# jlk9/MPAS-Ocean.jl

Measured on AMD Instinct MI355X. Metric: cell-updates/sec per RK4 step, higher is better.
Workload: dtype f64

## Files before the change

include/moka_hip.h:

```cpp
#ifndef MOKA_HIP_H
#define MOKA_HIP_H
#include <stdint.h>

#ifdef __cplusplus
extern "C" {
#endif

typedef struct moka_ctx   moka_ctx;
typedef struct moka_plan  moka_plan;
typedef struct moka_mesh  moka_mesh;
typedef struct moka_state moka_state;

typedef enum {
    MOKA_OK = 0,
    MOKA_ERR_ARG = -1,
    MOKA_ERR_HIP = -2,
    MOKA_ERR_NO_DEVICE = -3,
    MOKA_ERR_ALLOC = -4,
    MOKA_ERR_UNSUPPORTED = -5,
    MOKA_ERR_COMM = -6
} moka_status;

typedef enum {
    MOKA_ORDER_DEFAULT = 0,
// ... 112 lines not shown
int  moka_state_upload(moka_state *st, int field, int time_level, const double *host);
int  moka_state_download(moka_state *st, int field, int time_level, double *host);

int  moka_state_download_rows(moka_state *st, int field, int time_level, int64_t nRows, const int32_t *rows, double *host);

int  moka_state_array_address(moka_state *st, int field, int time_level, uint64_t *address);

int  moka_state_optimize_placement(moka_state *st, int max_tries, double *ms_before, double *ms_after);
typedef struct { int32_t field; double ms_old, ms_new; int32_t kept; } moka_placement_trial;
int  moka_state_placement_log(const moka_state *st, int32_t capacity, moka_placement_trial *out, int32_t *n);
int64_t moka_state_placement_launches(const moka_state *st);

int moka_advance_time_levels(moka_state *st, int flags);
int moka_diagnostic_compute(moka_state *st, int flags);
int moka_compute_normal_velocity_tendency(moka_state *st, int flags);
int moka_compute_layer_thickness_tendency(moka_state *st, int flags);
int moka_tendencies(moka_state *st);
int moka_step_fe(moka_state *st, double dt, int flags);
int moka_step_rk4(moka_state *st, double dt);
int moka_run(moka_state *st, int integrator, double dt, int64_t nsteps, int flags);
int moka_sum_sq(moka_state *st, int field, int time_level, double *out);

typedef struct moka_halo moka_halo;
int  moka_ctx_streams(moka_ctx *ctx, void **compute_stream, void **comm_stream);
int  moka_mesh_permutation(const moka_mesh *mesh, int kind, int32_t *new_to_old);
int  moka_mesh_class_ranges(const moka_mesh *mesh, int32_t capacity, int32_t *nClasses, int32_t *patchStart,
                            int32_t *cellStart, int32_t *edgeStart);
int  moka_halo_create(moka_state *st, int32_t nNeighbors, const int32_t *sendCells, const int64_t *sendCellOff,
                      const int32_t *sendEdges, const int64_t *sendEdgeOff, const int32_t *recvCells,
                      const int64_t *recvCellOff, const int32_t *recvEdges, const int64_t *recvEdgeOff,
                      int32_t nPatchesBoundary, int32_t nPatchesOwned, moka_halo **out);
void moka_halo_destroy(moka_halo *h);
int  moka_halo_buffer_elems(const moka_halo *h, int64_t *sendElems, int64_t *recvElems);
int  moka_halo_pack(moka_halo *h, int what, void *sendbuf_device);
int  moka_halo_unpack(moka_halo *h, int what, const void *recvbuf_device);

typedef struct {
    unsigned char ipc[15][64];
    uint64_t ptr[15];
    uint64_t flagPtr;
    char     shmName[64];
    int32_t  dstCell, dstEdge;
    int32_t  nCells, nEdges;
    int32_t  slot;
    int32_t  nNeighbors, pid, device, stateBytes, nVertLevels;
} moka_halo_peer_info;
int  moka_halo_set_overlap(moka_halo *h, int mode);
int  moka_halo_set_acquire(moka_halo *h, int on);
int  moka_halo_pack_fields(moka_halo *h, const void *uField, const void *hField, const void *sField, void *sendbuf);
int  moka_halo_unpack_fields(moka_halo *h, void *uField, void *hField, void *sField, const void *recvbuf);
int  moka_halo_direct_available(const moka_halo *h);
int  moka_halo_export(moka_halo *h, int32_t nbr, int32_t shared, moka_halo_peer_info *out);
int  moka_halo_connect(moka_halo *h, int32_t nbr, const moka_halo_peer_info *peer, int32_t shared);
int  moka_halo_push_begin(moka_halo *h, int what);
int  moka_halo_push_signal(moka_halo *h);
int  moka_halo_push_wait(moka_halo *h, double timeout_s);

int  moka_halo_set_stream_flags(moka_halo *h, int on);

typedef struct {
    int64_t steps, exchanges, boundary_launches, interior_launches;
    double host_step_ms, host_signal_wait_ms, host_flag_store_ms, host_wait_ms, boundary_launch_ms, interior_launch_ms;
} moka_halo_stats;
int  moka_halo_stats_enable(moka_halo *h, int on);
int  moka_halo_stats_read(moka_halo *h, moka_halo_stats *out);

int  moka_rk4_dist_begin(moka_halo *h, double dt);
int  moka_rk4_dist_stage(moka_halo *h, int stage, int part);
int  moka_rk4_dist_parts_available(const moka_halo *h);
int  moka_rk4_dist_stage_launch(moka_halo *h, int stage);
int  moka_rk4_dist_end(moka_halo *h);
typedef int (*moka_transport_fn)(void *user, int what, void *sendbuf_device, void *recvbuf_device);
int  moka_rk4_dist_step(moka_halo *h, double dt, moka_transport_fn transport, void *user, void *sendbuf_device,
                        void *recvbuf_device, double timeout_s);
int  moka_fe_dist_launch(moka_halo *h, double dt, int flags, int part);
int  moka_fe_dist_end(moka_halo *h);
int  moka_fe_dist_step(moka_halo *h, double dt, int flags, moka_transport_fn transport, void *user, void *sendbuf_device,
                       void *recvbuf_device, double timeout_s);

int moka_kernel_variant_available(int variant);
int moka_set_kernel_variant(moka_ctx *ctx, int variant);
int moka_set_tuning(int key, int value);
int moka_get_tuning(int key, int *value);
int moka_state_rk4_streams(const moka_state *st);
int moka_stage_timing(moka_ctx *ctx, int enable);
int moka_stage_timing_read(moka_ctx *ctx, double ms[4], int64_t *steps);
int moka_ctx_pci_bus_id(moka_ctx *ctx, char *buf, int32_t len);
int moka_mark(moka_ctx *ctx);
int moka_marks_reset(moka_ctx *ctx);
int moka_marks_read(moka_ctx *ctx, int64_t capacity, double *ms, int64_t *n);
int moka_bw_probe(moka_ctx *ctx, int64_t bytes, int iters, double gbs[4]);
int moka_bw_probe_streams(moka_ctx *ctx, int iters, double *gbs);
int moka_bw_probe_reread(moka_ctx *ctx, int64_t region, int reps, int iters, double *gbs);
int moka_bw_probe_gather_big(moka_ctx *ctx, int64_t bytes, int iters, double *gbs);
int moka_last_fe_path(const moka_state *st);
int moka_fe_lazy_pending(const moka_state *st);

int  moka_set_nonlinear(moka_state *st, int on);
int  moka_set_viscosity_del2(moka_state *st, double viscDel2);
int  moka_set_viscosity_del4(moka_state *st, double viscDel4, const double *meshScalingDel4);
int  moka_state_del4_path(const moka_state *st);

int  moka_set_tracers(moka_state *st, int32_t nTracers);
int  moka_tracer_upload(moka_state *st, int32_t j, int time_level, const double *host);
int  moka_tracer_download(moka_state *st, int32_t j, int time_level, double *host);
int  moka_state_tracer_path(const moka_state *st);
int  moka_set_tracer_diffusion(moka_state *st, const double *kappa);
int  moka_tracer_diffusion(const moka_state *st, int32_t j, double *out);
int  moka_set_tracer_biharmonic(moka_state *st, const double *kappa4);
int  moka_tracer_biharmonic(const moka_state *st, int32_t j, double *out);
int  moka_tracer_source_upload(moka_state *st, int32_t j, const double *host);
int  moka_tracer_source_download(moka_state *st, int32_t j, double *host);
int  moka_tracer_has_source(const moka_state *st, int32_t j, int *out);
int  moka_set_tracer_vertical_diffusion(moka_state *st, const double *kappaV);
int  moka_tracer_vertical_diffusion(const moka_state *st, int32_t j, double *out);
int  moka_state_tracer_vmix_path(const moka_state *st);
int  moka_tracer_vertical_field_upload(moka_state *st, int32_t j, const double *host);
int  moka_tracer_vertical_field_download(moka_state *st, int32_t j, double *host);
int  moka_tracer_has_vertical_field(const moka_state *st, int32_t j, int *out);

int  moka_set_vertical_viscosity(moka_state *st, double nuV, double bottomDrag);
int  moka_vertical_viscosity(const moka_state *st, double *nuV, double *bottomDrag);
int  moka_surface_stress_upload(moka_state *st, const double *host);
int  moka_surface_stress_download(moka_state *st, double *host);
int  moka_has_surface_stress(const moka_state *st, int *out);
int  moka_state_momentum_vmix_path(const moka_state *st);
int  moka_vertical_viscosity_field_upload(moka_state *st, const double *host);
int  moka_vertical_viscosity_field_download(moka_state *st, double *host);
int  moka_has_vertical_viscosity_field(const moka_state *st, int *out);

typedef struct moka_tracer_tape moka_tracer_tape;
int  moka_tracer_tape_create(moka_state *st, int64_t capacity_steps, moka_tracer_tape **out);
void moka_tracer_tape_destroy(moka_tracer_tape *t);
int  moka_step_rk4_tracer_taped(moka_tracer_tape *t, double dt);
int  moka_tracer_tape_steps(const moka_tracer_tape *t, int64_t *n);
int  moka_tracer_adjoint_seed(moka_tracer_tape *t, int32_t j, const double *host);
int  moka_tracer_adjoint_sweep(moka_tracer_tape *t);
int  moka_tracer_adjoint_download(moka_tracer_tape *t, int32_t j, double *host);
int  moka_tracer_adjoint_path(const moka_tracer_tape *t);
int  moka_tracer_adjoint_vmix_path(const moka_tracer_tape *t);
int  moka_tracer_adjoint_want_source_gradient(moka_tracer_tape *t, int32_t j, int on);
int  moka_tracer_adjoint_source_download(moka_tracer_tape *t, int32_t j, double *host);
enum { MOKA_TRACER_GRAD_KAPPA = 1, MOKA_TRACER_GRAD_KAPPA4 = 2 };
int  moka_tracer_adjoint_want_diffusivity_gradient(moka_tracer_tape *t, int32_t j, int what, int on);
int  moka_tracer_adjoint_diffusivity_gradient(moka_tracer_tape *t, int32_t j, int what, double *out);
int  moka_tracer_adjoint_diffusivity_density_download(moka_tracer_tape *t, int32_t j, int what, double *host);
int  moka_tracer_adjoint_want_vertical_gradient(moka_tracer_tape *t, int32_t j, int on);
int  moka_tracer_adjoint_vertical_gradient(moka_tracer_tape *t, int32_t j, double *out);
enum { MOKA_VGRAD_INTERFACE = 0, MOKA_VGRAD_CELL = 1, MOKA_VGRAD_PROFILE = 2 };
int  moka_tracer_adjoint_vertical_density_download(moka_tracer_tape *t, int32_t j, int view, double *host);

typedef struct moka_tape moka_tape;
int  moka_tape_create(moka_state *st, int64_t capacity_steps, moka_tape **out);
void moka_tape_destroy(moka_tape *t);
int  moka_step_fe_taped(moka_tape *t, double dt, int flags);
int  moka_step_rk4_taped(moka_tape *t, double dt);
int  moka_adjoint_seed_sum_sq_ssh(moka_tape *t);
int  moka_adjoint_sweep(moka_tape *t);
int  moka_tape_record_rk4(moka_tape *t, int slot, int what);
int  moka_tape_commit_rk4(moka_tape *t, double dt);
int  moka_adjoint_rk4_stage_fields(moka_tape *t, int stage, void **fieldU, void **fieldH, void **scratchS);
int  moka_adjoint_rk4_stage(moka_tape *t, int stage);
int  moka_adjoint_rk4_stage_part(moka_tape *t, int stage, int part);
int  moka_adjoint_rk4_parts_available(const moka_tape *t);
int  moka_adjoint_rk4_stage_out_fields(moka_tape *t, int stage, void **fieldU, void **fieldH, void **scratchS);
int  moka_tape_record_fe(moka_tape *t, int flags, int after);
// ... 26 lines not shown
```

mpas-ocean.jl_amd/csrc/api.hip:

```cpp
#include <hip/hip_runtime.h>

#include <algorithm>
#include <atomic>
#include <climits>
#include <cmath>
#include <cstdio>
#include <cstdlib>
#include <cstring>
#include <map>
#include <new>
#include <string>
#include <utility>
#include <vector>

#include "state.hpp"

namespace moka {

void fill_mesh_info(const Plan &p, moka_mesh_info *info);

struct TuningEntry {
    int mask, max;
    std::atomic<int> value;
    TuningEntry(int def, int m, int x) : mask(m), max(x), value(def) {}
    bool accepts(int v) const { return mask ? (v & ~mask) == 0 : v >= 0 && v <= max; }
};
static TuningEntry g_tuning[] = {
    {0, 0, -1},
    {1 << 0, 0x7f | 1 << 10 | 1 << 11, 0},
    {1, 0, 1},
    {1, 0, 1},
    {1, 0, 1},
    {0, 0, 3},
    {0, 0, INT_MAX},
    {0, 0, 1},
    {1 << 0 | 1 << 1 | 1 << 7, 0xf | 7 << 7 | 1 << 16, 0},
    {1, 0, 1},
};
constexpr int N_TUNING = sizeof(g_tuning) / sizeof(g_tuning[0]);

int tuning(TuningKey key) { return g_tuning[key].value.load(); }

}

namespace mk {

int fail(moka_ctx *ctx, int code, const std::string &msg)
{
    set_error(msg);
    if (ctx) ctx->err = msg;
    return code;
}

int lanes_per_column(int K)
{
    int l = 1;
    while (l < K && l < 64) l <<= 1;
    return l;
}

int h2d(moka_ctx *ctx, void *dst, const void *src, size_t bytes)
{
    if (!bytes) return MOKA_OK;
    HIPCHK(ctx, hipMemcpyAsync(dst, src, bytes, hipMemcpyHostToDevice, ctx->stream));
    HIPCHK(ctx, hipStreamSynchronize(ctx->stream));
    return MOKA_OK;
}

int ensure_op_bufs(moka_mesh *m)
{
    const Plan &p = m->plan;
    const size_t need = (size_t)p.K * std::max(p.nE, std::max(p.nC, p.nV));
    if (m->opBufElems >= need) return MOKA_OK;
    for (auto &b : m->opBuf) {
        if (b) HIPCHK(m->ctx, hipFree(b));
        b = nullptr;
    }
    for (auto &b : m->opBuf) HIPCHK(m->ctx, hipMalloc((void **)&b, need * sizeof(double)));
    m->opBufElems = need;
    return MOKA_OK;
}

const int32_t *perm_of(const moka_mesh *m, int kind)
{
    return kind == MOKA_CELL ? m->dev.cellN2O : kind == MOKA_EDGE ? m->dev.edgeN2O : m->dev.vertN2O;
}

int put_rows(moka_mesh *m, double *dst, const double *host, int kind, int64_t n, int K, bool f32)
{
    int rc = ensure_op_bufs(m);
    if (rc) return rc;
    hipStream_t s = m->ctx->stream;
    HIPCHK(m->ctx, hipMemcpyAsync(m->opBuf[2], host, (size_t)n * K * sizeof(double), hipMemcpyHostToDevice, s));
    if (f32) HIPCHK(m->ctx, launch_permute_rows_f32(dst, m->opBuf[2], perm_of(m, kind), n, K, 1, s));
    else HIPCHK(m->ctx, launch_permute_rows(dst, m->opBuf[2], perm_of(m, kind), n, K, 1, s));
    HIPCHK(m->ctx, hipStreamSynchronize(s));
    return MOKA_OK;
}

int get_rows(moka_mesh *m, double *host, const double *src, int kind, int64_t n, int K, bool f32)
{
    int rc = ensure_op_bufs(m);
    if (rc) return rc;
    hipStream_t s = m->ctx->stream;
    if (f32) HIPCHK(m->ctx, launch_permute_rows_f32(m->opBuf[2], src, perm_of(m, kind), n, K, 0, s));
    else HIPCHK(m->ctx, launch_permute_rows(m->opBuf[2], src, perm_of(m, kind), n, K, 0, s));
    HIPCHK(m->ctx, hipMemcpyAsync(host, m->opBuf[2], (size_t)n * K * sizeof(double), hipMemcpyDeviceToHost, s));
    HIPCHK(m->ctx, hipStreamSynchronize(s));
    return MOKA_OK;
}

}

using namespace mk;

extern "C" {

const char *moka_version(void) { return "moka-hip 0.1.0 (gfx950)"; }

// ... 169 lines not shown
            else bestGather = std::max(bestGather, (double)((2 * half) / rowB * rowB) / ((double)ms * 1e-3) / 1e9);
        }
    gbs[0] = bestCopy; gbs[1] = bestRead; gbs[2] = sumCopy / iters; gbs[3] = bestGather;
    return MOKA_OK;
}

int moka_bw_probe_streams(moka_ctx *ctx, int iters, double *gbs)
{
    if (!ctx || !gbs || iters < 1) return fail(ctx, MOKA_ERR_ARG, "NULL argument or iters < 1");
    if (!ctx->bwBuf || ctx->bwBytes < ((size_t)5 << 20)) return fail(ctx, MOKA_ERR_ARG, "moka_bw_probe first: it owns the buffer");
    HIPCHK(ctx, hipSetDevice(ctx->device));
    hipStream_t s = ctx->stream;
    const int64_t n = (int64_t)(ctx->bwBytes / 5 / 16);
    double best = 0.0;
    for (int i = 0; i < iters; ++i) {
        HIPCHK(ctx, hipEventRecord(ctx->ev0, s));
        HIPCHK(ctx, launch_bw_streams(ctx->bwBuf, (int64_t)ctx->bwBytes, s));
        HIPCHK(ctx, hipEventRecord(ctx->ev1, s));
        HIPCHK(ctx, hipEventSynchronize(ctx->ev1));
        float ms = 0.f;
        HIPCHK(ctx, hipEventElapsedTime(&ms, ctx->ev0, ctx->ev1));
        best = std::max(best, (double)(5 * 16 * n) / ((double)ms * 1e-3) / 1e9);
    }
    HIPCHK(ctx, hipMemsetAsync(ctx->bwBuf, 0x5A, ctx->bwBytes + 64, s));
    *gbs = best;
    return MOKA_OK;
}

int moka_bw_probe_reread(moka_ctx *ctx, int64_t region, int reps, int iters, double *gbs)
{
    if (!ctx || !gbs || iters < 1 || reps < 1) return fail(ctx, MOKA_ERR_ARG, "NULL argument or iters / reps < 1");
    if (!ctx->bwBuf || region < ((int64_t)1 << 20) || (size_t)region > ctx->bwBytes) return fail(ctx, MOKA_ERR_ARG, "moka_bw_probe first: it owns the buffer (region must fit it)");
    HIPCHK(ctx, hipSetDevice(ctx->device));
    hipStream_t s = ctx->stream;
    unsigned char *a = static_cast<unsigned char *>(ctx->bwBuf);
    uint32_t *sink = reinterpret_cast<uint32_t *>(a + ctx->bwBytes);
    region &= ~(int64_t)4095;
    double best = 0.0;
    HIPCHK(ctx, launch_bw_read(a, region, sink, ctx->nCUs, s));
    for (int i = 0; i < iters; ++i) {
        HIPCHK(ctx, hipEventRecord(ctx->ev0, s));
        for (int r = 0; r < reps; ++r) HIPCHK(ctx, launch_bw_read(a, region, sink, ctx->nCUs, s));
        HIPCHK(ctx, hipEventRecord(ctx->ev1, s));
        HIPCHK(ctx, hipEventSynchronize(ctx->ev1));
        float ms = 0.f;
        HIPCHK(ctx, hipEventElapsedTime(&ms, ctx->ev0, ctx->ev1));
        best = std::max(best, (double)region * reps / ((double)ms * 1e-3) / 1e9);
    }
    *gbs = best;
    return MOKA_OK;
}

int moka_bw_probe_gather_big(moka_ctx *ctx, int64_t bytes, int iters, double *gbs)
{
    if (!ctx || !gbs || iters < 1 || bytes < ((int64_t)1 << 24)) return fail(ctx, MOKA_ERR_ARG, "NULL argument, iters < 1 or less than 16 MiB");
    HIPCHK(ctx, hipSetDevice(ctx->device));
    hipStream_t s = ctx->stream;
    void *buf = nullptr;
    hipError_t e = hipMalloc(&buf, (size_t)bytes + 64);
    if (e != hipSuccess) return fail(ctx, MOKA_ERR_ALLOC, std::string("big gather probe: hipMalloc: ") + hipGetErrorString(e));
    const uint32_t rowB = 480;
    const int64_t nRows = bytes / rowB, nFetch = nRows / 4;
    uint32_t *sink = reinterpret_cast<uint32_t *>(static_cast<unsigned char *>(buf) + bytes);
    double best = 0.0;
    hipError_t rc = hipMemsetAsync(buf, 0x5A, (size_t)bytes + 64, s);
    for (int i = 0; i < iters && rc == hipSuccess; ++i) {
        if ((rc = hipEventRecord(ctx->ev0, s)) != hipSuccess) break;
        if ((rc = launch_bw_gather_n(buf, nRows, rowB, nFetch, sink, ctx->nCUs, s)) != hipSuccess) break;
        if ((rc = hipEventRecord(ctx->ev1, s)) != hipSuccess) break;
        if ((rc = hipEventSynchronize(ctx->ev1)) != hipSuccess) break;
        float ms = 0.f;
        if ((rc = hipEventElapsedTime(&ms, ctx->ev0, ctx->ev1)) != hipSuccess) break;
        best = std::max(best, (double)nFetch * rowB / ((double)ms * 1e-3) / 1e9);
    }
    (void)hipStreamSynchronize(s);
    (void)hipFree(buf);
    HIPCHK(ctx, rc);
    *gbs = best;
    return MOKA_OK;
}

int moka_set_tuning(int key, int value)
{
    if (key < 1 || key >= N_TUNING) return fail(nullptr, MOKA_ERR_ARG, "unknown tuning key");
    if (!g_tuning[key].accepts(value)) return fail(nullptr, MOKA_ERR_ARG, "tuning key " + std::to_string(key) + ": value names no kernel instance");
    g_tuning[key].value.store(value);
    return MOKA_OK;
}

int moka_get_tuning(int key, int *value)
{
    if (!value) return fail(nullptr, MOKA_ERR_ARG, "value is NULL");
    if (key < 1 || key >= N_TUNING) return fail(nullptr, MOKA_ERR_ARG, "unknown tuning key");
    *value = g_tuning[key].value.load();
    return MOKA_OK;
}

int moka_kernel_variant_available(int variant)
{
    return variant == 0 || variant == 3 || variant == 4 || variant == 11;
}

int moka_set_kernel_variant(moka_ctx *ctx, int variant)
{
    if (!ctx) return fail(nullptr, MOKA_ERR_ARG, "ctx is NULL");
    if (variant < 0 || variant > 14) return fail(ctx, MOKA_ERR_ARG, "variant must be 0..14");
    if (!moka_kernel_variant_available(variant))
        return fail(ctx, MOKA_ERR_UNSUPPORTED, "this kernel variant was an experiment of rounds 1-3 and no longer exists (0, 3, 4, 11 do)");
    ctx->variant = variant;
    return MOKA_OK;
}

int moka_mesh_create(moka_ctx *ctx, const moka_mesh_desc *desc, moka_mesh **out)
{
    if (!ctx || !out) return fail(ctx, MOKA_ERR_ARG, "NULL argument");
    *out = nullptr;
    moka_mesh *m = new (std::nothrow) moka_mesh();
    if (!m) return fail(ctx, MOKA_ERR_ALLOC, "out of host memory");
    m->ctx = ctx;
    m->mem.ctx = ctx;
    int rc;
    try {
        rc = build_plan(desc, m->plan);
    } catch (const std::bad_alloc &) {
        rc = fail(ctx, MOKA_ERR_ALLOC, "out of host memory while building the mesh plan");
    }
    if (rc != MOKA_OK) {
        ctx->err = moka::get_error();
        delete m;
        return rc;
    }
    const Plan &p = m->plan;
    if (p.ME > 8 || p.ME2 > 14) {
        delete m;
        return fail(ctx, MOKA_ERR_UNSUPPORTED, "cells with more than 8 edges are not supported by the gfx950 kernels");
    }
    HIPCHK(ctx, hipSetDevice(ctx->device));
    MeshDev &d = m->dev;
    d.nC = p.nC; d.nE = p.nE; d.nV = p.nV; d.K = p.K; d.ME = p.ME; d.ME2 = p.ME2; d.VD = p.VD; d.nPatches = p.nPatches;
    d.tailPatch = -1;
    m->lpc = lanes_per_column(p.K);
#define UP(field)                                                \
    if ((rc = m->mem.upload(p.field, &d.field)) != MOKA_OK) {   \
        moka_mesh_destroy(m);                                    \
        return rc;                                               \
    }
    UP(patchCellStart) UP(patchEdgeStart) UP(patchVertStart)
    UP(eoc) UP(coc) UP(mltc) UP(sdv) UP(invArea) UP(areaCell) UP(rsum)
    UP(ehdr) UP(eoe) UP(woe) UP(gInvDc) UP(dcEdge) UP(dvEdge) UP(fEdge)
    UP(eov) UP(cv) UP(cellN2O) UP(edgeN2O) UP(vertN2O)
    UP(leoe) UP(cRec) UP(eRec) UP(feoe) UP(vRec) UP(rowStart) UP(rowEdge)
    if (p.nlOk) { UP(voe) UP(cov) UP(kite) UP(invAreaTri) UP(fVertex) UP(keCoef) UP(invDc) UP(keoc) UP(rowVoe) }
    if (p.nl5Ok) { UP(pvStart) UP(pvList) UP(lvoe) }
#undef UP
    d.maxPV = p.nl5Ok ? p.maxPV : 0;
    if (!p.nl5Ok) { d.pvStart = nullptr; d.pvList = nullptr; d.lvoe = nullptr; }
    d.CI = p.CI; d.EI = p.EI;
    m->colOk = p.colOk;

    d.maxRows = p.maxRows; d.maxOwnE = p.maxOwnE; d.maxOwnC = p.maxOwnC;
    d.maxOwnV = p.maxOwnV;
    if (p.vRec.empty()) d.vRec = nullptr;
    *out = m;
    return MOKA_OK;
}

void moka_mesh_destroy(moka_mesh *mesh)
{
    if (!mesh) return;
    (void)hipSetDevice(mesh->ctx->device);
    (void)hipStreamSynchronize(mesh->ctx->stream);
    mesh->mem.release_all();
    for (auto b : mesh->opBuf)
        if (b) (void)hipFree(b);
    delete mesh;
}
// ... 192 lines not shown
```

mpas-ocean.jl_amd/csrc/api_state.hip:

```cpp
#include <hip/hip_runtime.h>

#include <algorithm>
#include <cmath>
#include <climits>
#include <cstdint>
#include <mutex>
#include <new>
#include <string>
#include <unordered_set>
#include <utility>
#include <vector>

#include "state.hpp"
#include "tapes.hpp"

namespace mk {

static std::mutex g_liveMutex;
static std::unordered_set<const moka_state *> g_liveStates;
void state_attach(moka_state *st, bool halo)
{
    std::lock_guard<std::mutex> lk(g_liveMutex);
    if (g_liveStates.count(st)) { ++st->attached; st->halos += halo; }
}
// ... 226 lines not shown
StageArgs fe_stage_args(moka_state *st, const FeArgs &a, int flags)
{
    StageArgs s{};
    s.pu = a.u; s.ph = a.h; s.ssh = a.ssh;
    s.pu_out = a.u_new; s.ph_out = a.h_new; s.ssh_out = a.ssh_new;
    s.a = a.dt;
    const bool stale = flags & MOKA_FE_STALE_HEDGE;
    const bool prev = stale && st->hEdgePrev && st->spare.ssh && a.h_new != st->lev[0].h && tuning(TUNE_FE_PREV);
    s.hEdgeOld = stale && !prev ? a.hEdgeOld : nullptr;
    s.hPrev = prev ? st->lev[0].h : nullptr;
    s.feMode = prev ? 6 : stale ? 4 : 5;
    s.areaCell = st->mesh->dev.areaCell;
    if (!fe_lean(st, flags)) {
        s.tendU = a.tendU; s.tendH = a.tendH;
        s.hEdgeNew = a.hEdgeNew; s.F = a.F; s.div = a.div;
    }
    if (stage_curl_fits(launch_bounds(st->mesh), st->f32)) { s.vort = a.vort; s.accumVort = (flags & MOKA_FE_ACCUM_VORT) ? 1 : 0; }
    return s;
}

static int materialize_fe(moka_state *st)
{
    const moka_mesh *mm = st->mesh;
    StageArgs g{};
    g.pu = st->lev[0].u; g.ph = st->lev[0].h; g.ssh = st->lev[0].ssh;
    g.feMode = st->feLazyStale ? 6 : 5;
    g.hPrev = st->feLazyStale ? st->spare.h : nullptr;
    g.tendU = st->tendU; g.tendH = st->tendH; g.F = st->F; g.div = st->div;
    g.hEdgeNew = st->hEdge[0];
    g.areaCell = mm->dev.areaCell;
    MeshDev dev = launch_bounds(mm);
    dev.tailPatch = -1;
    dev.patchBegin = 0; dev.nPatches = mm->plan.nPatchesLaunch;
    if (st->feLazyCount >= 0) {
        dev.patchBegin = st->feLazyBegin; dev.nPatches = st->feLazyCount;
    }
    if (dev.nPatches > 0)
        HIPCHK(st->ctx, st->f32 ? launch_stage_rec2c_f32(dev, g, st->ctx->stream) : launch_stage_rec2c(dev, g, st->ctx->stream));
    st->feLazy = false;
    st->feLazyCount = -1;
    return MOKA_OK;
}

int flush_lazy(moka_state *st, bool diag, bool tend)
{
    if ((diag || tend) && st->feLazy)
        if (int rc = materialize_fe(st)) return rc;
    if (diag && st->diagDirty && st->f32)
        return fail(st->ctx, MOKA_ERR_UNSUPPORTED,
                    "fp32-storage state: DiagnosticVars exist after Forward-Euler steps only (not after RK4 steps or uploads)");
    if (diag && st->diagDirty) {
        FeArgs a = fe_args(st, FE_FLUX | FE_DIV | FE_CURL | FE_HEDGE, 0, 0.0);
        a.nlev = st->mesh->plan.K;
        HIPCHK(st->ctx, launch_fe(st->mesh->dev, a, st->mesh->lpc, st->ctx->stream));
        std::swap(st->hEdge[0], st->hEdge[1]);
        st->diagDirty = false;
        st->hEdgePrev = false;
    }
    if (tend && st->tendDirty) {
        StageArgs g{};
        g.pu = st->lazyPu ? st->lazyPu : st->rk[0].u; g.ph = st->lazyPh ? st->lazyPh : st->rk[0].h; g.ssh = st->rk[0].ssh;
        g.tendU = st->tendU; g.tendH = st->tendH;
        HIPCHK(st->ctx, run_stage(st, g));
        st->tendDirty = false;
        st->lazyPu = st->lazyPh = nullptr; st->lazyOwner = nullptr;
    }
    return MOKA_OK;
}

bool is_diag_field(int f) { return f >= MOKA_F_LAYER_THICKNESS_EDGE && f <= MOKA_F_RELATIVE_VORTICITY; }
bool is_tend_field(int f) { return f == MOKA_F_TEND_NORMAL_VELOCITY || f == MOKA_F_TEND_LAYER_THICKNESS; }

static int make_ssh_consistent(moka_state *st, double *dst)
{
    const Plan &p = st->mesh->plan;
    if (st->f32)
        HIPCHK(st->ctx, launch_update_ssh_f32(st->mesh->dev, reinterpret_cast<const float *>(st->lev[1].h),
                                              reinterpret_cast<float *>(dst), p.K, st->mesh->lpc, st->ctx->stream));
    else
        HIPCHK(st->ctx, launch_update_ssh(st->mesh->dev, st->lev[1].h, dst, p.K, st->mesh->lpc, st->ctx->stream));
    return MOKA_OK;
}

StageArgs rk4_stage_args(moka_state *st, int s, double dt, const double *ssh0)
{
    const double a[3] = {dt / 2., dt / 2., dt};
    const double b[4] = {dt / 6., dt / 3., dt / 3., dt / 6.};
    LevelBufs &A = st->lev[1], &B = st->lev[0], &R1 = st->rk[0], &R2 = st->rk[1];
    StageArgs g{};
    g.nu_out = B.u; g.nh_out = B.h; g.b = b[s - 1];
    if (s == 1) {
        g.pu = A.u; g.ph = A.h; g.ssh = ssh0;
        g.pu_out = R1.u; g.ph_out = R1.h; g.ssh_out = R1.ssh; g.a = a[0];
    } else if (s == 2) {
        g.pu = R1.u; g.ph = R1.h; g.ssh = R1.ssh; g.cu = A.u; g.ch = A.h; g.nu_in = B.u; g.nh_in = B.h;
        g.pu_out = R2.u; g.ph_out = R2.h; g.ssh_out = R2.ssh; g.a = a[1];
    } else if (s == 3) {
        g.pu = R2.u; g.ph = R2.h; g.ssh = R2.ssh; g.cu = A.u; g.ch = A.h; g.nu_in = B.u; g.nh_in = B.h;
        g.pu_out = R1.u; g.ph_out = R1.h; g.ssh_out = R1.ssh; g.a = a[2];
    } else {
        g.pu = R1.u; g.ph = R1.h; g.ssh = R1.ssh; g.cu = A.u; g.ch = A.h; g.nu_in = B.u; g.nh_in = B.h;
        g.ssh_out = B.ssh; g.a = 0.0;
    }
    return g;
}

LevelBufs &rk4_stage_output(moka_state *st, int s)
{
    return s == 0 ? st->lev[1] : s == 5 ? fe_new_level(st) : s == 4 ? st->lev[0] : s == 2 ? st->rk[1] : st->rk[0];
}

int rk4_begin(moka_state *st, const double **ssh0)
{
    int rc = ensure_rk_bufs(st);
    if (rc) return rc;
    st->feLazy = false;
    *ssh0 = st->lev[1].ssh;
    if (!st->sshConsistent) {
        if ((rc = make_ssh_consistent(st, st->rk[1].ssh))) return rc;
        *ssh0 = st->rk[1].ssh;
    }
    return MOKA_OK;
}

void rk4_end(moka_state *st)
{
    std::swap(st->lev[0], st->lev[1]);
    std::swap(st->trPhi[0], st->trPhi[1]);
    st->sshConsistent = true;
    st->diagDirty = true;
    st->tendDirty = true;
    st->hEdgePrev = false;
    st->lazyPu = st->lazyPh = nullptr; st->lazyOwner = nullptr;
}

bool rk13_usable(const moka_state *st)
{
    if (!tuning(TUNE_RK13) || st->f32) return false;
    if (st->nTracers > 0) return false;
    if (st->nonlinear && st->viscDel4 != 0.0) return false;
    const moka_mesh *mm = st->mesh;
    if (mm->plan.nPatchesLaunch != mm->plan.nPatches) return false;
    if (st->nonlinear)
        return nl_stage_is_nl5(mm->dev, mm->lpc, mm->plan.ldsOk, nl_form(st->ctx));
    return default_stage_kernels(st) && rec2c_supported(launch_bounds(mm));
}

StageArgs rk13_stage_args(moka_state *st, int s, double dt, const double *ssh0)
{
    LevelBufs &A = st->lev[1], &B = st->lev[0], &R1 = st->rk[0], &R2 = st->rk[1];
    StageArgs g{};
    if (s == 1) {
        g.pu = A.u; g.ph = A.h; g.ssh = ssh0;
        g.pu_out = R1.u; g.ph_out = R1.h; g.ssh_out = R1.ssh; g.a = dt / 2.; g.rkMode = 7;
    } else if (s == 2) {
        g.pu = R1.u; g.ph = R1.h; g.ssh = R1.ssh; g.cu = A.u; g.ch = A.h;
        g.pu_out = R2.u; g.ph_out = R2.h; g.ssh_out = R2.ssh; g.a = dt / 2.; g.rkMode = 8;
    } else if (s == 3) {
        g.pu = R2.u; g.ph = R2.h; g.ssh = R2.ssh; g.cu = A.u; g.ch = A.h;
        g.pu_out = B.u; g.ph_out = B.h; g.ssh_out = B.ssh; g.a = dt; g.rkMode = 8;
    } else {
        g.pu = B.u; g.ph = B.h; g.ssh = B.ssh; g.cu = A.u; g.ch = A.h;
        g.nu_in = R1.u; g.nh_in = R1.h; g.q3u = R2.u; g.q3h = R2.h;
        g.nu_out = R1.u; g.nh_out = R1.h; g.ssh_out = R1.ssh; g.b = dt / 6.; g.rkMode = 9;
    }
    return g;
}

void rk13_end(moka_state *st)
{
    const LevelBufs A = st->lev[1], B = st->lev[0], R1 = st->rk[0];
    st->lev[1] = R1;
    st->lev[0] = A;
    st->rk[0] = B;
    st->sshConsistent = true;
    st->diagDirty = true;
    st->tendDirty = true;
    st->hEdgePrev = false;
    st->lazyPu = st->lazyPh = nullptr; st->lazyOwner = nullptr;
}

int momentum_vmix(moka_state *st, double *u, const double *h, double dt)
{
    const Plan &p = st->mesh->plan;
    MomVmixArgs a{};
    a.nE = p.nE; a.K = p.K; a.ehdr = st->mesh->dev.ehdr; a.u = u; a.h = h;
    a.tau = st->momTau && st->momTauOn ? st->momTau : nullptr;
    a.dt = dt; a.nu = mom_vmix_nu(st); a.drag = st->momDrag; a.scratch = st->momScratch;
    a.fld = mom_vmix_field(st);
    if (p.K < 2 && a.drag == 0.0 && !a.tau) return MOKA_OK;
    const bool generic = st->ctx->variant == 3;
    HIPCHK(st->ctx, launch_momentum_vmix(a, generic, st->ctx->stream));
    st->momVmixPath = momentum_vmix_form(p.K, generic);
    return MOKA_OK;
}

int step_rk4(moka_state *st, double dt, moka_tracer_tape *rec)
{
    HIPCHK(st->ctx, hipSetDevice(st->ctx->device));
    const bool vmix = st->nTracers > 0 && st->trKappaVDev != nullptr;
    if (vmix && dt < 0.0) return fail(st->ctx, MOKA_ERR_ARG, "vertical tracer diffusion: dt must be >= 0 (the implicit solve is not reversible in time)");
    const bool mvmix = mom_vmix_on(st);
    if (mvmix && dt < 0.0) return fail(st->ctx, MOKA_ERR_ARG, "vertical momentum mixing: dt must be >= 0 (the implicit solve is not reversible in time)");
    const double *ssh0 = nullptr;
    int rc = rk4_begin(st, &ssh0);
    if (rc) return rc;
    moka_ctx *c = st->ctx;
    hipStreamCaptureStatus cap = hipStreamCaptureStatusNone;
    (void)hipStreamIsCapturing(c->stream, &cap);
    const bool timed = c->stageTiming && cap == hipStreamCaptureStatusNone;
    auto stamp = [&]() -> hipError_t {
        if (c->evUsed == c->evPool.size()) {
            hipEvent_t e = nullptr;
            if (hipError_t er = hipEventCreate(&e); er != hipSuccess) return er;
            c->evPool.push_back(e);
        }
        return hipEventRecord(c->evPool[c->evUsed++], c->stream);
    };
    const bool s13 = rk13_usable(st);
    for (int s = 1; s <= 4; ++s) {
        if (timed) HIPCHK(c, stamp());
        const StageArgs g = s13 ? rk13_stage_args(st, s, dt, ssh0) : rk4_stage_args(st, s, dt, ssh0);
        HIPCHK(c, run_stage(st, g));
        if (st->nTracers > 0) HIPCHK(c, tracer_stage(st, s, g));
        if (s == 4 && vmix && st->mesh->plan.K >= 2 && dt != 0.0)
            if ((rc = tracer_vmix(st->mesh, c, st->nTracers, g.nh_out, st->trPhi[0], st->trKappaVDev, st->trVfDev, dt, st->trVmixScratch, false, &st->vmixPath))) return rc;
        if (s == 4 && mvmix && dt != 0.0)
            if ((rc = momentum_vmix(st, g.nu_out, g.nh_out, dt))) return rc;
        if (rec) {
            const Plan &p = st->mesh->plan;
            const size_t nEK = (size_t)p.K * p.nE, nCK = (size_t)p.K * p.nC;
            HIPCHK(c, hipMemcpyAsync(rec->pu + nEK * (4 * rec->n + s - 1), g.pu, nEK * sizeof(double), hipMemcpyDeviceToDevice, c->stream));
            HIPCHK(c, hipMemcpyAsync(rec->ph + nCK * (4 * rec->n + s - 1), g.ph, nCK * sizeof(double), hipMemcpyDeviceToDevice, c->stream));
            if (s == 4) HIPCHK(c, hipMemcpyAsync(rec->hn + nCK * rec->n, g.nh_out, nCK * sizeof(double), hipMemcpyDeviceToDevice, c->stream));
            const double *pphi = s == 1 ? st->trPhi[1] : st->trProv[s == 3 ? 1 : 0];
            const size_t nF = rec->kgTracer.size();
            for (size_t f = 0; f < nF; ++f)
                HIPCHK(c, hipMemcpyAsync(rec->kgP + nCK * ((4 * rec->n + s - 1) * nF + f), pphi + nCK * rec->kgTracer[f], nCK * sizeof(double),
                                         hipMemcpyDeviceToDevice, c->stream));
            const size_t nV = rec->vgTracer.size();
            for (size_t f = 0; s == 4 && f < nV; ++f)
                HIPCHK(c, hipMemcpyAsync(rec->vgP + nCK * (rec->n * nV + f), st->trPhi[0] + nCK * rec->vgTracer[f], nCK * sizeof(double),
                                         hipMemcpyDeviceToDevice, c->stream));
        }
    }
    if (timed) HIPCHK(c, stamp());
    if (s13) rk13_end(st);
    else rk4_end(st);
    return MOKA_OK;
}


}

using namespace mk;

extern "C" {

int moka_state_create(moka_ctx *ctx, moka_mesh *mesh, moka_state **out)
{
    if (!ctx || !mesh || !out) return fail(ctx, MOKA_ERR_ARG, "NULL argument");
    *out = nullptr;
    moka_state *st = new (std::nothrow) moka_state();
    if (!st) return fail(ctx, MOKA_ERR_ALLOC, "out of host memory");
    st->ctx = ctx;
    st->mem.ctx = ctx;
    st->mesh = mesh;
    const Plan &p = mesh->plan;
    HIPCHK(ctx, hipSetDevice(ctx->device));
    const size_t nEK = (size_t)p.K * p.nE, nCK = (size_t)p.K * p.nC, nVK = (size_t)p.K * p.nV;
    st->f32 = p.stateBytes == 4;
    const MeshDev launchDev = launch_bounds(mesh);
    if (st->f32 && !stage_f32_supported(launchDev)) {
        delete st;
        return fail(ctx, MOKA_ERR_UNSUPPORTED,
                    "fp32-storage state: needs nVertLevels % 4 == 0, nVertLevels <= 128, fields below 4 GiB and patches whose "
                    "records + own u rows fit 64 KB of LDS (smaller patch_cells)");
    }
    const size_t sb = st->f32 ? 4 : 8;
    int rc = MOKA_OK;
    auto A = [&](double **q, size_t n, size_t eb = 8) { if (rc == MOKA_OK) rc = st->mem.alloc(q, n, eb); };
    for (auto &l : st->lev) { A(&l.ssh, p.nC, sb); A(&l.u, nEK, sb); A(&l.h, nCK, sb); }
    A(&st->hEdge[0], nEK, sb); A(&st->hEdge[1], nEK, sb);
    A(&st->F, nEK, sb); A(&st->div, nCK, sb); A(&st->vort, nVK, sb);
    A(&st->tendU, nEK, sb); A(&st->tendH, nCK, sb);
    A(&st->scalar, 2);
    if (rc != MOKA_OK) { moka_state_destroy(st); return rc; }
    st->phys[0] = st->lev[0]; st->phys[1] = st->lev[1];
    HIPCHK(ctx, hipStreamSynchronize(ctx->stream));
    {
        std::lock_guard<std::mutex> lk(g_liveMutex);
        g_liveStates.insert(st);
    }
    *out = st;
    return MOKA_OK;
}

void moka_state_destroy(moka_state *st)
{
    if (!st) return;
    {
        std::lock_guard<std::mutex> lk(g_liveMutex);
        g_liveStates.erase(st);
    }
    (void)hipSetDevice(st->ctx->device);
// ... 570 lines not shown
```

mpas-ocean.jl_amd/csrc/inspect.hip:

```cpp
#include <algorithm>

#include "state.hpp"

using namespace mk;

namespace {

template <class T>
__global__ __launch_bounds__(256) void k_gather_rows(double *dst, const T *src, const int32_t *rows, int64_t n, int K)
{
    const int64_t total = n * K;
    for (int64_t i = (int64_t)blockIdx.x * 256 + threadIdx.x; i < total; i += (int64_t)gridDim.x * 256) {
        const int64_t r = i / K;
        const int k = (int)(i - r * K);
        dst[i] = (double)src[(int64_t)rows[r] * K + k];
    }
}

}

extern "C" int moka_state_download_rows(moka_state *st, int field, int time_level, int64_t nRows, const int32_t *rows, double *host)
{
    if (!st || (nRows > 0 && (!rows || !host)) || nRows < 0) return fail(st ? st->ctx : nullptr, MOKA_ERR_ARG, "NULL argument or nRows < 0");
    moka_ctx *c = st->ctx;
    const Plan &p = st->mesh->plan;
    HIPCHK(c, hipSetDevice(c->device));
    const bool diag = field >= MOKA_F_LAYER_THICKNESS_EDGE && field <= MOKA_F_RELATIVE_VORTICITY;
    const bool tend = field == MOKA_F_TEND_NORMAL_VELOCITY || field == MOKA_F_TEND_LAYER_THICKNESS;
    if (int rc = flush_lazy(st, diag, tend)) return rc;
    const double *src = nullptr;
    int kind = MOKA_CELL, K = p.K;
    if (time_level == 2 || time_level == 3) {
        const LevelBufs &b = st->rk[time_level - 2];
        if (!b.ssh) return fail(c, MOKA_ERR_ARG, "the RK4 provisional states exist after the first RK4 step only");
        switch (field) {
            case MOKA_F_SSH: src = b.ssh; K = 1; break;
            case MOKA_F_NORMAL_VELOCITY: src = b.u; kind = MOKA_EDGE; break;
            case MOKA_F_LAYER_THICKNESS: src = b.h; break;
            default: return fail(c, MOKA_ERR_ARG, "time_level 2 / 3 (RK4 provisional states): prognostic fields only");
        }
    } else if (time_level == 0 || time_level == 1) {
        switch (field) {
            case MOKA_F_SSH: src = st->lev[time_level].ssh; K = 1; break;
            case MOKA_F_NORMAL_VELOCITY: src = st->lev[time_level].u; kind = MOKA_EDGE; break;
            case MOKA_F_LAYER_THICKNESS: src = st->lev[time_level].h; break;
            case MOKA_F_LAYER_THICKNESS_EDGE: src = st->hEdge[0]; kind = MOKA_EDGE; break;
            case MOKA_F_THICKNESS_FLUX: src = st->F; kind = MOKA_EDGE; break;
            case MOKA_F_VELOCITY_DIV_CELL: src = st->div; break;
            case MOKA_F_RELATIVE_VORTICITY: src = st->vort; kind = MOKA_VERTEX; break;
            case MOKA_F_TEND_NORMAL_VELOCITY: src = st->tendU; kind = MOKA_EDGE; break;
            case MOKA_F_TEND_LAYER_THICKNESS: src = st->tendH; break;
            default: return fail(c, MOKA_ERR_ARG, "unknown field id");
        }
    } else {
        return fail(c, MOKA_ERR_ARG, "time_level must be 0 (previous), 1 (current), 2 or 3 (RK4 provisional states)");
    }
    if (!src) return fail(c, MOKA_ERR_ARG, "field not allocated");
    if (nRows == 0) return MOKA_OK;
    const int64_t nEnt = kind == MOKA_CELL ? p.nC : kind == MOKA_EDGE ? p.nE : p.nV;
    const std::vector<int32_t> &o2n = kind == MOKA_CELL ? p.cellO2N : kind == MOKA_EDGE ? p.edgeO2N : p.vertO2N;
    std::vector<int32_t> lib(nRows);
    for (int64_t i = 0; i < nRows; ++i) {
        if (rows[i] < 0 || rows[i] >= nEnt) return fail(c, MOKA_ERR_ARG, "row id out of range");
        lib[i] = o2n[rows[i]];
    }
    int32_t *dRows = nullptr;
    double *dOut = nullptr;
    auto done = [&](int rc) {
        if (dRows) (void)hipFree(dRows);
        if (dOut) (void)hipFree(dOut);
        return rc;
    };
    if (hipMalloc((void **)&dRows, (size_t)nRows * sizeof(int32_t)) != hipSuccess ||
        hipMalloc((void **)&dOut, (size_t)nRows * K * sizeof(double)) != hipSuccess) {
        (void)hipGetLastError();
        return done(fail(c, MOKA_ERR_ALLOC, "moka_state_download_rows: hipMalloc failed"));
    }
    hipStream_t s = c->stream;
    hipError_t e = hipMemcpyAsync(dRows, lib.data(), (size_t)nRows * sizeof(int32_t), hipMemcpyHostToDevice, s);
    if (e == hipSuccess) {
        const unsigned blocks = (unsigned)std::min<int64_t>((nRows * K + 255) / 256, 16384);
        if (st->f32) hipLaunchKernelGGL(k_gather_rows<float>, dim3(blocks), dim3(256), 0, s, dOut, reinterpret_cast<const float *>(src), dRows, nRows, K);
        else hipLaunchKernelGGL(k_gather_rows<double>, dim3(blocks), dim3(256), 0, s, dOut, src, dRows, nRows, K);
        e = hipGetLastError();
    }
    if (e == hipSuccess) e = hipMemcpyAsync(host, dOut, (size_t)nRows * K * sizeof(double), hipMemcpyDeviceToHost, s);
    if (e == hipSuccess) e = hipStreamSynchronize(s);
    if (e != hipSuccess) return done(fail(c, MOKA_ERR_HIP, std::string("moka_state_download_rows: ") + hipGetErrorString(e)));
    return done(MOKA_OK);
}

extern "C" int moka_state_array_address(moka_state *st, int field, int time_level, uint64_t *address)
{
    if (!st || !address) return fail(st ? st->ctx : nullptr, MOKA_ERR_ARG, "NULL argument");
    if (time_level < 0 || time_level > 3 || field < MOKA_F_SSH || field > MOKA_F_LAYER_THICKNESS)
        return fail(st->ctx, MOKA_ERR_ARG, "prognostic fields, time_level 0..3");
    const LevelBufs &b = time_level < 2 ? st->lev[time_level] : st->rk[time_level - 2];
    const double *q = field == MOKA_F_SSH ? b.ssh : field == MOKA_F_NORMAL_VELOCITY ? b.u : b.h;
    *address = (uint64_t)(uintptr_t)q;
    return MOKA_OK;
}
```

mpas-ocean.jl_amd/csrc/kernels.hip:

```cpp
#include <mutex>
#include <set>
#include <utility>

#include "kernels_common.hpp"

namespace moka {


template <int ME, int ME2, int MODE, int NT = BLOCK>
__global__ __launch_bounds__(NT) void k_stage_rec2c(const ColMesh m, const StageArgs a, int maxOwnE, int maxOwnC)
{
    extern __shared__ __align__(16) unsigned char smem[];
    const int pl_ = patch_of_block(m.nPatches);
    if (pl_ >= m.nPatches) return;
    const int p = m.pairEnd ? m.patchBegin + 2 * pl_ : (m.tailPlus1 && pl_ == m.nPatches - 1) ? m.tailPlus1 - 1 : pl_ + m.patchBegin;
    const int pEnd = m.pairEnd ? (p + 2 < m.pairEnd ? p + 2 : m.pairEnd) : p + 1;
    constexpr int NG = NT / 32;
    const int tid = threadIdx.x;
    const int grp = tid >> 5, l = tid & 31;
    const int K = m.K, K2 = K >> 1;
    const uint32_t voff = (uint32_t)l * 16u, rowB = (uint32_t)K * 8u;
    const RecLds L = rec_carve(smem, m, ME, ME2, maxOwnE, maxOwnC);
    const size_t recBytes = ((size_t)maxOwnE * (2 * ME2 + 1) * 8 + (size_t)maxOwnC * (ME + 2) * 8 +
                             ((size_t)maxOwnE * m.EI + (size_t)maxOwnC * m.CI) * 4 + 15) & ~(size_t)15;
    double2 *ubuf2 = reinterpret_cast<double2 *>(smem + recBytes);
    const unsigned char *ubytes = reinterpret_cast<const unsigned char *>(ubuf2) + voff;
    const int c0 = cptr(m.patchCellStart)[p], c1 = cptr(m.patchCellStart)[pEnd];
    const int e0 = cptr(m.patchEdgeStart)[p], e1 = cptr(m.patchEdgeStart)[pEnd];
    const int nOwnC = c1 - c0, nOwnE = e1 - e0;
    const uint32_t e0B = (uint32_t)e0 * rowB, nOwnB = (uint32_t)nOwnE * rowB;
    double *Lvw = reinterpret_cast<double *>(smem + recBytes + (size_t)maxOwnE * rowB);
    uint32_t *Lvo = reinterpret_cast<uint32_t *>(Lvw + (size_t)m.maxOwnV * 3);
    constexpr bool LEAN = MODE >= 10;
    constexpr int BASE = LEAN ? MODE - 5 : MODE;
    constexpr bool FE = BASE >= 4 && BASE <= 6, STALE = BASE == 4, PREV = BASE == 6;
    int v0 = 0, nOwnV = 0;
    if constexpr (FE) {
        if (a.vort) {
            v0 = cptr(m.patchVertStart)[p];
            nOwnV = cptr(m.patchVertStart)[p + 1] - v0;
        }
    }

    {
        const double2 *src = reinterpret_cast<const double2 *>(a.pu) + (size_t)e0 * K2;
        const int nU = nOwnE * K2, nER = nOwnE * m.EI, nW = nOwnE * ME2, nCR = nOwnC * m.CI, nS = nOwnC * ME;
        constexpr int UU = 6, UE = 3, UW = 2;
        double2 vU[UU];
        uint32_t vE[UE], vC;
        double vW[UW], vF[UW], vG, vS, vA, vR;
#pragma unroll
        for (int j = 0; j < UU; ++j) vU[j] = (tid + j * NT < nU) ? src[tid + j * NT] : make_double2(0.0, 0.0);
#pragma unroll
        for (int j = 0; j < UE; ++j) vE[j] = (tid + j * NT < nER) ? m.eRec[(size_t)e0 * m.EI + tid + j * NT] : 0u;
#pragma unroll
        for (int j = 0; j < UW; ++j) {
            vW[j] = (tid + j * NT < nW) ? m.woe[(size_t)e0 * ME2 + tid + j * NT] : 0.0;
            vF[j] = (tid + j * NT < nW) ? m.feoe[(size_t)e0 * ME2 + tid + j * NT] : 0.0;
        }
        vG = tid < nOwnE ? m.gInvDc[e0 + tid] : 0.0;
        vC = tid < nCR ? m.cRec[(size_t)c0 * m.CI + tid] : 0u;
        vS = tid < nS ? m.sdv[(size_t)c0 * ME + tid] : 0.0;
        vA = tid < nOwnC ? m.invArea[c0 + tid] : 0.0;
        vR = tid < nOwnC ? m.rsum[c0 + tid] : 0.0;
        uint32_t vVo = 0u;
        double vVw = 0.0;
        if constexpr (FE) {
            if (tid < nOwnV * 4) vVo = m.vRec[(size_t)v0 * 4 + tid];
            if (tid < nOwnV * 3) vVw = m.cv[(size_t)v0 * 3 + tid];
        }
#pragma unroll
        for (int j = 0; j < UU; ++j) if (tid + j * NT < nU) ubuf2[tid + j * NT] = vU[j];
#pragma unroll
        for (int j = 0; j < UE; ++j) if (tid + j * NT < nER) L.eRec[tid + j * NT] = vE[j];
#pragma unroll
        for (int j = 0; j < UW; ++j)
            if (tid + j * NT < nW) {
                L.woe[tid + j * NT] = vW[j];
                L.feoe[tid + j * NT] = vF[j];
            }
        if (tid < nOwnE) L.g[tid] = vG;
        if (tid < nCR) L.cRec[tid] = vC;
        if (tid < nS) L.sdv[tid] = vS;
        if (tid < nOwnC) {
            L.invA[tid] = vA;
            L.rsum[tid] = vR;
        }
        if constexpr (FE) {
            if (tid < nOwnV * 4) Lvo[tid] = vVo;
            if (tid < nOwnV * 3) Lvw[tid] = vVw;
            for (int i = tid + NT; i < nOwnV * 4; i += NT) Lvo[i] = m.vRec[(size_t)v0 * 4 + i];
            for (int i = tid + NT; i < nOwnV * 3; i += NT) Lvw[i] = m.cv[(size_t)v0 * 3 + i];
        }
        for (int i = tid + UU * NT; i < nU; i += NT) ubuf2[i] = src[i];
        for (int i = tid + UE * NT; i < nER; i += NT) L.eRec[i] = m.eRec[(size_t)e0 * m.EI + i];
        for (int i = tid + UW * NT; i < nW; i += NT) {
            L.woe[i] = m.woe[(size_t)e0 * ME2 + i];
            L.feoe[i] = m.feoe[(size_t)e0 * ME2 + i];
        }
        for (int i = tid + NT; i < nOwnE; i += NT) L.g[i] = m.gInvDc[e0 + i];
        for (int i = tid + NT; i < nCR; i += NT) L.cRec[i] = m.cRec[(size_t)c0 * m.CI + i];
        for (int i = tid + NT; i < nS; i += NT) L.sdv[i] = m.sdv[(size_t)c0 * ME + i];
        for (int i = tid + NT; i < nOwnC; i += NT) {
            L.invA[i] = m.invArea[c0 + i];
            L.rsum[i] = m.rsum[c0 + i];
        }
    }
    __syncthreads();

    const int k0 = 2 * l;
    const bool act = k0 < K;
    const lds_bytes_t ubytesL = (lds_bytes_t)ubytes;
    const glb_bytes_t puG = (glb_bytes_t)a.pu;
    const uint32_t ldsU = (uint32_t)(size_t)ubytesL;
    auto urow_addr = [&](uint32_t off, bool &cached) -> uint32_t {
        const uint32_t loc = off - e0B;
        cached = loc < nOwnB;
        return ldsU + (cached ? loc : 0u);
    };

    double2 pA = make_double2(0.0, 0.0), pB = pA, pD = pA, pE = pA;
    double pS = 0.0;
    uint32_t pOff = 0;
    int pC = 0;
    bool pend = false;
    auto flush_cell = [&]() {
        if (act) {
            if constexpr (MODE == 0) gstore2o(a.tendH, pOff, pA);
            if constexpr (MODE == 1 || MODE == 2) {
                gstore2o(a.ph_out, pOff, pA);
                gstore2o(a.nh_out, pOff, pB);
            }
            if constexpr (MODE == 3 || MODE == 9) gstore2o(a.nh_out, pOff, pB);
            if constexpr (MODE == 7 || MODE == 8) gstore2o(a.ph_out, pOff, pA);
            if constexpr (LEAN) gstore2o(a.ph_out, pOff, pA);
            if constexpr (FE && !LEAN) {
                if (a.ph_out) gstore2o(a.ph_out, pOff, pA);
                if (a.tendH) gstore2o(a.tendH, pOff, pB);
                if (a.div) gstore2o(a.div, pOff, pD);
            }
        }
        if constexpr (MODE != 0)
            if (l == 0 && (!FE || LEAN || a.ssh_out)) a.ssh_out[pC] = pS;
    };
#pragma nounroll
    for (int ci = grp; ci < nOwnC; ci += NG) {
        const int c = c0 + ci;
        const uint32_t *r = L.cRec + (size_t)ci * m.CI;
        const double *rs = L.sdv + (size_t)ci * ME;
        const uint32_t mask = r[2 * ME], all = r[2 * ME + 1];
        const double invA = L.invA[ci];
        const uint32_t own = (uint32_t)c * rowB + voff;
        double2 hc = make_double2(0.0, 0.0), uv[ME], hv[ME], cur = hc, nin = hc, hpc = hc, q3 = hc;
        if (act) {
            bool cached[ME];
            uint32_t ad[ME], goff[ME];
            v4u_t raw[ME];
            hc = gload2(a.ph, own);
            if constexpr (PREV) hpc = gload2(a.hPrev, own);
#pragma unroll
            for (int i = 0; i < ME; ++i) {
                const uint32_t off = r[i];
                hv[i] = STALE ? gload2(a.hEdgeOld, off + voff) : gload2(PREV ? a.hPrev : a.ph, r[ME + i] + voff);
                ad[i] = urow_addr(off, cached[i]);
                goff[i] = off + voff;
                asm("" : "+v"(goff[i]));
            }
            lds_burst<ME>(raw, ad);
#pragma unroll
            for (int i = 0; i < ME; ++i) {
                uv[i] = __builtin_bit_cast(double2, raw[i]);
                if (!cached[i]) uv[i] = glb_row2(puG + goff[i]);
            }
            if constexpr (MODE == 2 || MODE == 8 || MODE == 9) cur = gload2(a.ch, own);
            if constexpr (MODE == 2 || MODE == 3 || MODE == 9) nin = gload2(a.nh_in, own);
            if constexpr (MODE == 9) q3 = gload2(a.q3h, own);
        }
        double area = 1.0;
        if constexpr (FE && !LEAN) if (a.div) area = a.areaCell[c];
        __builtin_amdgcn_s_waitcnt(0x0F70);
        if (pend) flush_cell();
        double2 t = make_double2(0.0, 0.0);
        const bool plain = __builtin_amdgcn_ballot_w64(!(mask == (1u << ME) - 1u && all)) == 0;
        double2 dv = make_double2(0.0, 0.0);
        const double2 hself = PREV ? hpc : hc;
        auto hE = [&](int i) { return STALE ? hv[i] : make_double2(0.5 * (hself.x + hv[i].x), 0.5 * (hself.y + hv[i].y)); };
        if (plain) {
            if (act) {
#pragma unroll
                for (int i = 0; i < ME; ++i) {
                    const double2 he = hE(i);
                    t.x += uv[i].x * he.x * rs[i] * invA;
                    t.y += uv[i].y * he.y * rs[i] * invA;
                    if constexpr (FE && !LEAN) {
                        dv.x -= uv[i].x * rs[i];
                        dv.y -= uv[i].y * rs[i];
                    }
                }
            }
        } else if (act) {
#pragma unroll
            for (int i = 0; i < ME; ++i) {
                const int ml = all ? K : cptr(m.mltc)[(size_t)c * ME + i];
                const bool on = (mask >> i) & 1u;
                const double2 he = hE(i);
                const double dx = uv[i].x * he.x * rs[i] * invA;
                const double dy = uv[i].y * he.y * rs[i] * invA;
                if (on && k0 < ml) t.x += dx;
                if (on && k0 + 1 < ml) t.y += dy;
                if constexpr (FE && !LEAN) {
                    if (on) {
                        dv.x -= uv[i].x * rs[i];
                        dv.y -= uv[i].y * rs[i];
                    }
                }
            }
        }
        double2 hs = make_double2(0.0, 0.0);
        if (act) {
            if constexpr (MODE == 0) pA = t;
            if constexpr (MODE == 1 || MODE == 2) {
                const double2 hcur = MODE == 2 ? cur : hc;
                const double2 nb = MODE == 2 ? nin : hcur;
                hs = make_double2(hcur.x + a.a * t.x, hcur.y + a.a * t.y);
                pA = hs;
                pB = make_double2(nb.x + a.b * t.x, nb.y + a.b * t.y);
            }
            if constexpr (MODE == 3) {
                hs = make_double2(nin.x + a.b * t.x, nin.y + a.b * t.y);
                pB = hs;
            }
            if constexpr (MODE == 7 || MODE == 8) {
                const double2 hcur = MODE == 8 ? cur : hc;
                hs = make_double2(hcur.x + a.a * t.x, hcur.y + a.a * t.y);
                pA = hs;
            }
            if constexpr (MODE == 9) {
                hs = make_double2(rk13_combine(cur.x, nin.x, q3.x, hc.x, a.b, t.x), rk13_combine(cur.y, nin.y, q3.y, hc.y, a.b, t.y));
                pB = hs;
            }
            if constexpr (FE) {
                hs = make_double2(hc.x + a.a * t.x, hc.y + a.a * t.y);
                pA = hs;
                if constexpr (!LEAN) {
                    pB = t;
                    if (a.div) pD = make_double2(dv.x / area, dv.y / area);
                }
            }
        }
        if constexpr (MODE != 0) {
#pragma unroll
            for (int sft = 16; sft >= 1; sft >>= 1) {
                const double ox = __shfl_xor(hs.x, sft, 32), oy = __shfl_xor(hs.y, sft, 32);
                hs = make_double2(hs.x + ox, hs.y + oy);
            }
            pS = (hs.x + hs.y) - L.rsum[ci];
        }
        pOff = own;
        pC = c;
        pend = true;
    }
    if (pend) flush_cell();
    pend = false;
    auto flush_edge = [&]() {
        if (act) {
            if constexpr (MODE == 0) gstore2o(a.tendU, pOff, pA);
            if constexpr (MODE == 1 || MODE == 2) {
                gstore2o(a.pu_out, pOff, pA);
                gstore2o(a.nu_out, pOff, pB);
            }
            if constexpr (MODE == 3 || MODE == 9) gstore2o(a.nu_out, pOff, pB);
            if constexpr (MODE == 7 || MODE == 8) gstore2o(a.pu_out, pOff, pA);
            if constexpr (LEAN) gstore2o(a.pu_out, pOff, pA);
            if constexpr (FE && !LEAN) {
                if (a.pu_out) gstore2o(a.pu_out, pOff, pA);
                if (a.tendU) gstore2o(a.tendU, pOff, pB);
                if (a.F) gstore2o(a.F, pOff, pD);
                if (a.hEdgeNew) gstore2o(a.hEdgeNew, pOff, pE);
            }
        }
    };

#pragma nounroll
    for (int ei = grp; ei < nOwnE; ei += NG) {
        const int e = e0 + ei;
        const uint32_t *r = L.eRec + (size_t)ei * m.EI;
        const double *rw = L.woe + (size_t)ei * ME2;
        const double *rf = L.feoe + (size_t)ei * ME2;
        const uint32_t mask = r[ME2 + 2];
        const int mlt = (int)r[ME2 + 3];
        const double g = L.g[ei];
        const uint32_t own = (uint32_t)e * rowB + voff;
        double sv = 0.0;
        double2 uv[ME2], cur = make_double2(0.0, 0.0), nin = cur, hx = cur, hy = cur, hEo = cur, q3 = cur;
        if (act) {
            bool cached[ME2];
            uint32_t ad[ME2], goff[ME2];
            v4u_t raw[ME2];
#pragma unroll
            for (int i = 0; i < ME2; ++i) {
                const uint32_t off = r[i];
                ad[i] = urow_addr(off, cached[i]);
                goff[i] = off + voff;
                asm("" : "+v"(goff[i]));
            }
            lds_burst<ME2>(raw, ad);
#pragma unroll
            for (int i = 0; i < ME2; ++i) {
                uv[i] = __builtin_bit_cast(double2, raw[i]);
                if (!cached[i]) uv[i] = glb_row2(puG + goff[i]);
            }
            if constexpr (MODE == 2 || MODE == 8 || MODE == 9) cur = gload2(a.cu, own);
            if constexpr (MODE == 2 || MODE == 3 || MODE == 9) nin = gload2(a.nu_in, own);
            if constexpr (MODE == 9) q3 = gload2(a.q3u, own);
            if constexpr (FE && !LEAN) {
                if (a.hEdgeNew || (MODE == 5 && a.F)) {
                    hx = gload2(a.ph, r[ME2] * rowB + voff);
                    hy = gload2(a.ph, r[ME2 + 1] * rowB + voff);
                }
                if (a.F) {
                    if constexpr (STALE) hEo = gload2(a.hEdgeOld, own);
                    if constexpr (PREV) {
                        const double2 px = gload2(a.hPrev, r[ME2] * rowB + voff), py = gload2(a.hPrev, r[ME2 + 1] * rowB + voff);
                        hEo = make_double2(0.5 * (px.x + py.x), 0.5 * (px.y + py.y));
                    }
                }
            }
        }
        if (l < 2) sv = a.ssh[r[ME2 + l]];
        __builtin_amdgcn_s_waitcnt(0x0F70);
        if (pend) flush_edge();
        const double ds = __shfl(sv, 1, 32) - __shfl(sv, 0, 32);
        const bool plain = __builtin_amdgcn_ballot_w64(!(mask == (1u << ME2) - 1u && mlt >= K)) == 0;
        if (act) {
            const bool ax = k0 < mlt, ay = k0 + 1 < mlt;
            double2 t = make_double2(0.0, 0.0);
            if (plain) {
                t.x -= g * ds;
                t.y -= g * ds;
#pragma unroll
                for (int i = 0; i < ME2; ++i) {
                    t.x += rw[i] * uv[i].x * rf[i];
                    t.y += rw[i] * uv[i].y * rf[i];
                }
            } else {
                if (ax) t.x -= g * ds;
                if (ay) t.y -= g * ds;
#pragma unroll
                for (int i = 0; i < ME2; ++i) {
                    const bool on = (mask >> i) & 1u;
                    const double px = rw[i] * uv[i].x * rf[i], py = rw[i] * uv[i].y * rf[i];
                    if (on && ax) t.x += px;
                    if (on && ay) t.y += py;
                }
            }
            if constexpr (MODE == 0) pA = t;
            if constexpr (MODE == 1) {
                const double2 up = ubuf2[(size_t)ei * K2 + l];
                pA = make_double2(up.x + a.a * t.x, up.y + a.a * t.y);
                pB = make_double2(up.x + a.b * t.x, up.y + a.b * t.y);
            }
            if constexpr (MODE == 2) {
                pA = make_double2(cur.x + a.a * t.x, cur.y + a.a * t.y);
                pB = make_double2(nin.x + a.b * t.x, nin.y + a.b * t.y);
            }
            if constexpr (MODE == 3) pB = make_double2(nin.x + a.b * t.x, nin.y + a.b * t.y);
            if constexpr (MODE == 7) {
                const double2 up = ubuf2[(size_t)ei * K2 + l];
                pA = make_double2(up.x + a.a * t.x, up.y + a.a * t.y);
            }
            if constexpr (MODE == 8) pA = make_double2(cur.x + a.a * t.x, cur.y + a.a * t.y);
            if constexpr (MODE == 9) {
                const double2 up = ubuf2[(size_t)ei * K2 + l];
                pB = make_double2(rk13_combine(cur.x, nin.x, q3.x, up.x, a.b, t.x), rk13_combine(cur.y, nin.y, q3.y, up.y, a.b, t.y));
            }
            if constexpr (LEAN) {
                const double2 up = ubuf2[(size_t)ei * K2 + l];
                pA = make_double2(up.x + a.a * t.x, up.y + a.a * t.y);
            }
            if constexpr (FE && !LEAN) {
                const double2 up = ubuf2[(size_t)ei * K2 + l];
                pE = make_double2(0.5 * (hx.x + hy.x), 0.5 * (hx.y + hy.y));
                const double2 hF = (STALE || PREV) ? hEo : pE;
                pD = make_double2(up.x * hF.x, up.y * hF.y);
                pA = make_double2(up.x + a.a * t.x, up.y + a.a * t.y);
                pB = t;
            }
        }
        pOff = own;
        pend = true;
    }
    if (pend) flush_edge();

    if constexpr (FE) {
#pragma nounroll
        for (int vi = grp; vi < nOwnV; vi += NG) {
            if (!act) continue;
            const uint32_t *rv = Lvo + (size_t)vi * 4;
            const double *wv = Lvw + (size_t)vi * 3;
            const uint32_t own = (uint32_t)(v0 + vi) * rowB + voff;
            bool cached[3];
            uint32_t ad[3], goff[3];
            v4u_t raw[3];
            double2 uv[3];
#pragma unroll
            for (int j = 0; j < 3; ++j) {
                const uint32_t off = rv[j];
                ad[j] = urow_addr(off, cached[j]);
                goff[j] = off + voff;
                asm("" : "+v"(goff[j]));
            }
            double2 c = a.accumVort ? gload2(a.vort, own) : make_double2(0.0, 0.0);
            lds_burst<3>(raw, ad);
#pragma unroll
            for (int j = 0; j < 3; ++j) {
                uv[j] = __builtin_bit_cast(double2, raw[j]);
                if (!cached[j]) uv[j] = glb_row2(puG + goff[j]);
            }
#pragma unroll
            for (int j = 0; j < 3; ++j) {
                c.x += wv[j] * uv[j].x;
                c.y += wv[j] * uv[j].y;
            }
            gstore2(a.vort, own, c);
        }
    }
}

struct d4 {
    double x, y, z, w;
};
__device__ __forceinline__ d4 widen4(float4 v) { return d4{(double)v.x, (double)v.y, (double)v.z, (double)v.w}; }
__device__ __forceinline__ float4 narrow4(d4 v) { return make_float4((float)v.x, (float)v.y, (float)v.z, (float)v.w); }
__device__ __forceinline__ float4 gload4f(const double *base, uint32_t off)
{
    return *reinterpret_cast<const float4 *>(reinterpret_cast<const char *>(base) + off);
}
__device__ __forceinline__ d4 gload4(const double *base, uint32_t off)
{
    return widen4(*reinterpret_cast<const float4 *>(reinterpret_cast<const char *>(base) + off));
}
__device__ __forceinline__ void gstore4(double *base, uint32_t off, d4 v)
{
    *reinterpret_cast<float4 *>(reinterpret_cast<char *>(base) + off) = narrow4(v);
}
__device__ __forceinline__ d4 axpy4(d4 x, double a, d4 t)
{
    return d4{x.x + a * t.x, x.y + a * t.y, x.z + a * t.z, x.w + a * t.w};
}
__device__ __forceinline__ d4 round4(d4 v) { return widen4(narrow4(v)); }

template <int ME, int ME2, int MODE, int NT = BLOCK, int WPE = 3>
__global__ __launch_bounds__(NT, WPE) void k_stage_rec2c_f32(const ColMesh m, const StageArgs a, int maxOwnE, int maxOwnC)
{
    extern __shared__ __align__(16) unsigned char smem[];
    const int pl_ = patch_of_block(m.nPatches);
    if (pl_ >= m.nPatches) return;
    const int p = (m.tailPlus1 && pl_ == m.nPatches - 1) ? m.tailPlus1 - 1 : pl_ + m.patchBegin;
    const int tid = threadIdx.x;
    const int K = m.K, K4 = K >> 2;
    const int EPW = 64 / K4, NG = (NT / 64) * EPW;
    const int lane = tid & 63, sub = lane / K4;
    const int l = lane - sub * K4, gbase = sub * K4;
    const bool lane_on = sub < EPW;
    const int grp = lane_on ? (tid >> 6) * EPW + sub : (1 << 28);
    auto gxor = [&](double v, int sft) -> double {
        const int pl = l ^ sft;
        const double o = __shfl(v, gbase + (pl < K4 ? pl : l), 64);
        return pl < K4 ? o : 0.0;
    };
    const uint32_t voff = (uint32_t)l * 16u, rowB = (uint32_t)K * 4u;
// ... 806 lines not shown
        }
#pragma unroll
        for (int j = 0; j < 4; ++j) acc ^= v[j].x ^ v[j].y ^ v[j].z ^ v[j].w;
    }
    if (acc == 0x9E3779B9u) *sink = acc;
}

__global__ __launch_bounds__(BLOCK) void k_bw_streams(bw_v4u *__restrict__ o1, bw_v4u *__restrict__ o2, const bw_v4u *__restrict__ a,
                                                     const bw_v4u *__restrict__ b, const bw_v4u *__restrict__ c, int64_t n)
{
    const int64_t i = (int64_t)blockIdx.x * BLOCK + threadIdx.x;
    if (i < n) {
        const bw_v4u x = a[i], y = b[i], z = c[i];
        o1[i] = x ^ y;
        o2[i] = x ^ z;
    }
}

hipError_t launch_bw_streams(void *buf, int64_t bytes, hipStream_t s)
{
    const int64_t n = bytes / 5 / 16;
    bw_v4u *p = static_cast<bw_v4u *>(buf);
    hipLaunchKernelGGL(k_bw_streams, dim3((unsigned)((n + BLOCK - 1) / BLOCK)), dim3(BLOCK), 0, s, p + 3 * n, p + 4 * n, p, p + n, p + 2 * n, n);
    return hipGetLastError();
}

hipError_t launch_bw_copy(void *dst, const void *src, int64_t bytes, int, hipStream_t s)
{
    const int64_t n = bytes / 16;
    hipLaunchKernelGGL(k_bw_copy, dim3((unsigned)((n + BLOCK - 1) / BLOCK)), dim3(BLOCK), 0, s, static_cast<bw_v4u *>(dst),
                       static_cast<const bw_v4u *>(src), n);
    return hipGetLastError();
}

hipError_t launch_bw_read(const void *src, int64_t bytes, uint32_t *sink, int, hipStream_t s)
{
    const int64_t n = bytes / 16;
    hipLaunchKernelGGL(k_bw_read, dim3((unsigned)((n + 4 * BLOCK - 1) / (4 * BLOCK))), dim3(BLOCK), 0, s, static_cast<const bw_v4u *>(src), n, sink);
    return hipGetLastError();
}

hipError_t launch_bw_gather(const void *src, int64_t bytes, uint32_t rowB, uint32_t *sink, int nCUs, hipStream_t s)
{
    const int64_t nRows = bytes / rowB;
    hipLaunchKernelGGL(k_bw_gather, dim3((unsigned)(nCUs * 16)), dim3(BLOCK), 0, s, static_cast<const unsigned char *>(src), nRows, rowB, nRows, sink);
    return hipGetLastError();
}

hipError_t launch_bw_gather_n(const void *src, int64_t nRows, uint32_t rowB, int64_t nFetch, uint32_t *sink, int nCUs, hipStream_t s)
{
    hipLaunchKernelGGL(k_bw_gather, dim3((unsigned)(nCUs * 16)), dim3(BLOCK), 0, s, static_cast<const unsigned char *>(src), nRows, rowB, nFetch, sink);
    return hipGetLastError();
}

template <int LPC>
static hipError_t launch_fe_lpc(const MeshDev &m, const FeArgs &a, hipStream_t s)
{
    const dim3 g(patch_grid(m)), b(BLOCK);
    if (m.ME == 6 && m.ME2 == 10) hipLaunchKernelGGL((k_fe<LPC, 6, 10>), g, b, 0, s, m, a);
    else if (m.ME == 8 && m.ME2 == 14) hipLaunchKernelGGL((k_fe<LPC, 8, 14>), g, b, 0, s, m, a);
    else if (m.ME <= 6 && m.ME2 <= 14) hipLaunchKernelGGL((k_fe<LPC, 6, 14>), g, b, 0, s, m, a);
    else return hipErrorInvalidValue;
    return hipGetLastError();
}


template <int ME, int ME2, int NT>
static bool launch_rec2c_nt(const ColMesh &m, const StageArgs &a, int mode, dim3 g, size_t lds, int mE, int mC, hipStream_t s)
{
    const dim3 b(NT);
    switch (mode) {
        case 0: hipLaunchKernelGGL((k_stage_rec2c<ME, ME2, 0, NT>), g, b, lds, s, m, a, mE, mC); return true;
        case 1: hipLaunchKernelGGL((k_stage_rec2c<ME, ME2, 1, NT>), g, b, lds, s, m, a, mE, mC); return true;
        case 2: hipLaunchKernelGGL((k_stage_rec2c<ME, ME2, 2, NT>), g, b, lds, s, m, a, mE, mC); return true;
        case 3: hipLaunchKernelGGL((k_stage_rec2c<ME, ME2, 3, NT>), g, b, lds, s, m, a, mE, mC); return true;
        case 4: hipLaunchKernelGGL((k_stage_rec2c<ME, ME2, 4, NT>), g, b, lds, s, m, a, mE, mC); return true;
        case 5: hipLaunchKernelGGL((k_stage_rec2c<ME, ME2, 5, NT>), g, b, lds, s, m, a, mE, mC); return true;
        case 6: hipLaunchKernelGGL((k_stage_rec2c<ME, ME2, 6, NT>), g, b, lds, s, m, a, mE, mC); return true;
        case 7: hipLaunchKernelGGL((k_stage_rec2c<ME, ME2, 7, NT>), g, b, lds, s, m, a, mE, mC); return true;
        case 8: hipLaunchKernelGGL((k_stage_rec2c<ME, ME2, 8, NT>), g, b, lds, s, m, a, mE, mC); return true;
        case 9: hipLaunchKernelGGL((k_stage_rec2c<ME, ME2, 9, NT>), g, b, lds, s, m, a, mE, mC); return true;
        case 10: hipLaunchKernelGGL((k_stage_rec2c<ME, ME2, 10, NT>), g, b, lds, s, m, a, mE, mC); return true;
        case 11: hipLaunchKernelGGL((k_stage_rec2c<ME, ME2, 11, NT>), g, b, lds, s, m, a, mE, mC); return true;
    }
    return false;
}

template <int ME, int ME2>
static bool launch_rec2c(const ColMesh &m, const StageArgs &a, int mode, dim3 g, dim3, size_t lds, int mE, int mC, hipStream_t s)
{
    if (m.nPatches <= 512) return launch_rec2c_nt<ME, ME2, 512>(m, a, mode, g, lds, mE, mC, s);
    return launch_rec2c_nt<ME, ME2, BLOCK>(m, a, mode, g, lds, mE, mC, s);
}

hipError_t raise_dyn_lds(std::initializer_list<const void *> fns, int bytes)
{
    static std::mutex mu;
    static std::set<std::pair<int, const void *>> done;
    int dev = 0;
    if (hipError_t e = hipGetDevice(&dev); e != hipSuccess) return e;
    std::lock_guard<std::mutex> lk(mu);
    for (const void *fn : fns) {
        if (done.count({dev, fn})) continue;
        if (hipError_t e = hipFuncSetAttribute(fn, hipFuncAttributeMaxDynamicSharedMemorySize, bytes); e != hipSuccess) return e;
        done.insert({dev, fn});
    }
    return hipSuccess;
}

template <int ME, int ME2>
static hipError_t launch_rec2c_pair(const ColMesh &m, const StageArgs &a, int mode, dim3 g, size_t lds, int mE, int mC, hipStream_t s)
{
    const dim3 b(512);
#define PAIR_CASE(M)                                                                                                   \
    case M:                                                                                                            \
        if (lds > 64 * 1024)                                                                                           \
            if (hipError_t e = raise_dyn_lds({(const void *)k_stage_rec2c<ME, ME2, M, 512>}, 160 * 1024); e != hipSuccess) \
                return e;                                                                                              \
        hipLaunchKernelGGL((k_stage_rec2c<ME, ME2, M, 512>), g, b, lds, s, m, a, mE, mC);                               \
        return hipGetLastError();
    switch (mode) {
        PAIR_CASE(0) PAIR_CASE(1) PAIR_CASE(2) PAIR_CASE(3) PAIR_CASE(7) PAIR_CASE(8) PAIR_CASE(9)
    }
#undef PAIR_CASE
    return hipErrorNotSupported;
}

size_t rec2c_lds_bytes(const MeshDev &md)
{
    return ((rec_lds_bytes(md) + 15) & ~(size_t)15) + (size_t)md.maxOwnE * md.K * 8 + 16;
}

static inline size_t vert_lds_bytes(const MeshDev &md) { return (size_t)md.maxOwnV * (3 * 8 + 4 * 4) + 16; }

bool stage_curl_fused(const MeshDev &md)
{
    return tuning(TUNE_CURL_FUSED) && md.vRec != nullptr && md.VD == 3 && md.patchVertStart != nullptr && md.maxOwnV > 0;
}

bool stage_curl_fits(const MeshDev &md, bool f32)
{
    if (!stage_curl_fused(md)) return false;
    const size_t rows = (size_t)md.maxOwnE * md.K * (f32 ? 4 : 8);
    const size_t lds = ((rec_lds_bytes(md) + 15) & ~(size_t)15) + rows + 16 + vert_lds_bytes(md) + 16;
    return f32 ? (stage_f32_supported(md) && lds <= 160 * 1024) : (rec2c_supported(md) && lds <= 64 * 1024);
}

static inline ColMesh col_mesh(const MeshDev &md, int nLaunch)
{
    return ColMesh{md.nC, md.nE, md.K, nLaunch, md.patchBegin, md.CI, md.EI, md.patchCellStart, md.patchEdgeStart,
                   md.cRec, md.eRec, md.mltc, md.sdv, md.invArea, md.rsum, md.woe, md.feoe, md.gInvDc, md.tailPatch >= 0 ? md.tailPatch + 1 : 0,
                   md.patchVertStart, md.vRec, md.cv, md.maxOwnV, 0};
}

bool rec2c_supported(const MeshDev &md)
{
    const bool shape = (md.ME == 6 && md.ME2 == 10) || (md.ME == 8 && md.ME2 == 14) || (md.ME <= 6 && md.ME2 <= 14);
    return md.cRec && md.eRec && md.K <= 64 && !(md.K & 1) && rec2c_lds_bytes(md) <= 64 * 1024 && md.maxOwnC >= 1 && md.maxOwnE >= 1 && shape;
}

hipError_t launch_stage_rec2c(const MeshDev &md, const StageArgs &a, hipStream_t s)
{
    const int nLaunch = md.nPatches + (md.tailPatch >= 0 ? 1 : 0);
    const dim3 g(8 * ((nLaunch + 7) / 8)), b(BLOCK);
    const ColMesh m = col_mesh(md, nLaunch);
    int mode = colp_mode(a);
    if (a.vort && (mode < 4 || !stage_curl_fused(md))) return hipErrorNotSupported;
    if (tuning(TUNE_FE_LEAN_INST) && colp_lean(a, mode)) mode += 5;
    const size_t lds = rec2c_lds_bytes(md) + (a.vort ? vert_lds_bytes(md) : 0);
    if (mode < 0 || md.K > 64 || (md.K & 1) || lds > 64 * 1024 || md.maxOwnC < 1 || md.maxOwnE < 1) return hipErrorNotSupported;
    const int pair = tuning(TUNE_PAIR);
    if (((pair >> mode) & 1) && md.tailPatch < 0 && (md.nPatches >= 4096 || ((pair >> 16) & 1)) && md.nPatches >= 2 &&
        md.ME == 6 && md.ME2 == 10) {
        MeshDev two = md;
        two.maxOwnE = 2 * md.maxOwnE; two.maxOwnC = 2 * md.maxOwnC;
        const size_t lds2 = rec2c_lds_bytes(two);
        if (2 * lds2 + 2048 <= 160 * 1024) {
            const int nPair = (md.nPatches + 1) / 2;
            ColMesh mp = col_mesh(md, nPair);
            mp.pairEnd = md.patchBegin + md.nPatches;
            const hipError_t e = launch_rec2c_pair<6, 10>(mp, a, mode, dim3(8 * ((nPair + 7) / 8)), lds2, two.maxOwnE, two.maxOwnC, s);
            if (e != hipErrorNotSupported) return e;
        }
    }
    bool ok = false;
    if (md.ME == 6 && md.ME2 == 10) ok = launch_rec2c<6, 10>(m, a, mode, g, b, lds, md.maxOwnE, md.maxOwnC, s);
    else if (md.ME == 8 && md.ME2 == 14) ok = launch_rec2c<8, 14>(m, a, mode, g, b, lds, md.maxOwnE, md.maxOwnC, s);
    else if (md.ME <= 6 && md.ME2 <= 14) ok = launch_rec2c<6, 14>(m, a, mode, g, b, lds, md.maxOwnE, md.maxOwnC, s);
    return ok ? hipGetLastError() : hipErrorNotSupported;
}

template <int ME, int ME2, int NT, int WPE>
static hipError_t launch_rec2c_f32_nt(const ColMesh &m, const StageArgs &a, int mode, dim3 g, size_t lds, int mE, int mC, hipStream_t s)
{
    if (lds > 64 * 1024) {
        const hipError_t e = raise_dyn_lds({(const void *)k_stage_rec2c_f32<ME, ME2, 0, NT, WPE>, (const void *)k_stage_rec2c_f32<ME, ME2, 1, NT, WPE>,
                                            (const void *)k_stage_rec2c_f32<ME, ME2, 2, NT, WPE>, (const void *)k_stage_rec2c_f32<ME, ME2, 3, NT, WPE>,
                                            (const void *)k_stage_rec2c_f32<ME, ME2, 4, NT, WPE>, (const void *)k_stage_rec2c_f32<ME, ME2, 5, NT, WPE>,
                                            (const void *)k_stage_rec2c_f32<ME, ME2, 6, NT, WPE>, (const void *)k_stage_rec2c_f32<ME, ME2, 10, NT, WPE>,
                                            (const void *)k_stage_rec2c_f32<ME, ME2, 11, NT, WPE>},
                                           160 * 1024);
        if (e != hipSuccess) return e;
    }
    const dim3 b(NT);
    switch (mode) {
        case 0: hipLaunchKernelGGL((k_stage_rec2c_f32<ME, ME2, 0, NT, WPE>), g, b, lds, s, m, a, mE, mC); return hipGetLastError();
        case 1: hipLaunchKernelGGL((k_stage_rec2c_f32<ME, ME2, 1, NT, WPE>), g, b, lds, s, m, a, mE, mC); return hipGetLastError();
        case 2: hipLaunchKernelGGL((k_stage_rec2c_f32<ME, ME2, 2, NT, WPE>), g, b, lds, s, m, a, mE, mC); return hipGetLastError();
        case 3: hipLaunchKernelGGL((k_stage_rec2c_f32<ME, ME2, 3, NT, WPE>), g, b, lds, s, m, a, mE, mC); return hipGetLastError();
        case 4: hipLaunchKernelGGL((k_stage_rec2c_f32<ME, ME2, 4, NT, WPE>), g, b, lds, s, m, a, mE, mC); return hipGetLastError();
        case 5: hipLaunchKernelGGL((k_stage_rec2c_f32<ME, ME2, 5, NT, WPE>), g, b, lds, s, m, a, mE, mC); return hipGetLastError();
        case 6: hipLaunchKernelGGL((k_stage_rec2c_f32<ME, ME2, 6, NT, WPE>), g, b, lds, s, m, a, mE, mC); return hipGetLastError();
        case 10: hipLaunchKernelGGL((k_stage_rec2c_f32<ME, ME2, 10, NT, WPE>), g, b, lds, s, m, a, mE, mC); return hipGetLastError();
        case 11: hipLaunchKernelGGL((k_stage_rec2c_f32<ME, ME2, 11, NT, WPE>), g, b, lds, s, m, a, mE, mC); return hipGetLastError();
    }
    return hipErrorNotSupported;
}

template <int ME, int ME2>
static hipError_t launch_rec2c_f32(const ColMesh &m, const StageArgs &a, int mode, dim3 g, size_t lds, int mE, int mC, hipStream_t s)
{
    if (((tuning(TUNE_F32_WIDE) >> mode) & 1) && 2 * lds <= 160 * 1024)
        return launch_rec2c_f32_nt<ME, ME2, 512, 4>(m, a, mode, g, lds, mE, mC, s);
    return launch_rec2c_f32_nt<ME, ME2, BLOCK, 3>(m, a, mode, g, lds, mE, mC, s);
}

bool stage_f32_supported(const MeshDev &md)
{
    const size_t lds = ((rec_lds_bytes(md) + 15) & ~(size_t)15) + (size_t)md.maxOwnE * md.K * 4 + 16;
    const bool shape = (md.ME == 6 && md.ME2 == 10) || (md.ME == 8 && md.ME2 == 14) || (md.ME <= 6 && md.ME2 <= 14);
    return md.cRec && md.eRec && md.K >= 4 && md.K <= 128 && (md.K & 3) == 0 && lds <= 160 * 1024 && md.maxOwnC >= 1 &&
           md.maxOwnE >= 1 && shape;
}

hipError_t launch_stage_rec2c_f32(const MeshDev &md, const StageArgs &a, hipStream_t s)
{
    const int nLaunch = md.nPatches + (md.tailPatch >= 0 ? 1 : 0);
    const dim3 g(8 * ((nLaunch + 7) / 8));
    const ColMesh m = col_mesh(md, nLaunch);
    int mode = colp_mode(a);
    if (mode < 0 || !stage_f32_supported(md)) return hipErrorNotSupported;
    if (a.vort && (mode < 4 || !stage_curl_fused(md))) return hipErrorNotSupported;
    if (tuning(TUNE_FE_LEAN_INST) && colp_lean(a, mode)) mode += 5;
    const size_t lds = ((rec_lds_bytes(md) + 15) & ~(size_t)15) + (size_t)md.maxOwnE * md.K * 4 + 16 + (a.vort ? vert_lds_bytes(md) + 16 : 0);
    if (lds > 160 * 1024) return hipErrorNotSupported;
    if (md.ME == 6 && md.ME2 == 10) return launch_rec2c_f32<6, 10>(m, a, mode, g, lds, md.maxOwnE, md.maxOwnC, s);
    if (md.ME == 8 && md.ME2 == 14) return launch_rec2c_f32<8, 14>(m, a, mode, g, lds, md.maxOwnE, md.maxOwnC, s);
    if (md.ME <= 6 && md.ME2 <= 14) return launch_rec2c_f32<6, 14>(m, a, mode, g, lds, md.maxOwnE, md.maxOwnC, s);
    return hipErrorNotSupported;
}

hipError_t launch_curl2(const MeshDev &m, const double *u, double *vort, bool accum, hipStream_t s)
{
    if (m.K > 64 || (m.K & 1) || (size_t)std::max(m.nE, m.nV) * m.K * 8 >= ((size_t)1 << 32)) return hipErrorNotSupported;
    if (m.VD == 3) hipLaunchKernelGGL((k_curl3<3>), dim3(patch_grid(m)), dim3(BLOCK), 0, s, m, u, vort, accum ? 1 : 0);
// ... 122 lines not shown
```

mpas-ocean.jl_amd/csrc/kernels.hpp:

```cpp
#pragma once
#include <hip/hip_runtime.h>

#include <initializer_list>

#include "moka_internal.hpp"

namespace moka {

struct StageArgs {
    const double *pu, *ph;
    const double *ssh;
    const double *cu, *ch;
    const double *nu_in, *nh_in;
    double *nu_out, *nh_out;
    double *pu_out, *ph_out;
    double *ssh_out;
    double *tendU, *tendH;
    double a, b;
    int feMode;
    const double *hEdgeOld;
    const double *hPrev;
    double *hEdgeNew, *F, *div;
    const double *areaCell;
    double *vort;
    int accumVort;
    int rkMode;
    const double *q3u, *q3h;
};

struct ColMesh {
    int32_t nC, nE, K, nPatches, patchBegin, CI, EI;
    const int32_t *patchCellStart, *patchEdgeStart;
    const uint32_t *cRec, *eRec;
    const int32_t *mltc;
    const double *sdv, *invArea, *rsum, *woe, *feoe, *gInvDc;
    int32_t tailPlus1;
    const int32_t *patchVertStart;
    const uint32_t *vRec;
    const double *cv;
    int32_t maxOwnV;
    int32_t pairEnd;
};

enum : int {
    FE_FLUX = 1, FE_DIV = 2, FE_CURL = 4, FE_HEDGE = 8, FE_TENDU = 16, FE_TENDH = 32, FE_UPDATE = 64,
    FE_TENDH_FROM_F = 128
};

struct FeArgs {
    int ops, flags, nlev;
    double dt;
    const double *u, *h, *ssh;
    const double *hEdgeOld;
    const double *Fin;
    double *hEdgeNew, *F, *div, *vort, *tendU, *tendH;
    double *u_new, *h_new, *ssh_new;
};

enum : int { OP_GRADIENT = 0, OP_INTERP = 1, OP_DIV_P1 = 2, OP_DIV_P2 = 3, OP_CURL = 4, OP_GRAD_T = 5, OP_DIV_T = 6, OP_CURL_T = 7 };

struct OpArgs {
    int op, nlev;
    const double *in;
    double *out;
    const double *in2 = nullptr;
    const int32_t *auxI = nullptr;
    const double *auxD = nullptr;
    int auxW = 0;
};

hipError_t launch_stage(const MeshDev &m, const StageArgs &a, int lpc, hipStream_t s);
hipError_t launch_stage_col(const MeshDev &m, const StageArgs &a, hipStream_t s);
hipError_t launch_stage_rec2c(const MeshDev &m, const StageArgs &a, hipStream_t s);
bool rec2c_supported(const MeshDev &m);
bool stage_curl_fused(const MeshDev &m);
bool stage_curl_fits(const MeshDev &m, bool f32);
bool stage_f32_supported(const MeshDev &m);
hipError_t launch_stage_rec2c_f32(const MeshDev &m, const StageArgs &a, hipStream_t s);

enum TuningKey : int {
    TUNE_F32_WIDE = 1,
    TUNE_FE_PREV = 2,
    TUNE_CURL_FUSED = 3,
    TUNE_FE_LEAN = 4,
    TUNE_NL_SHAPE = 5,
    TUNE_NL_CAP = 6,
    TUNE_RK13 = 7,
    TUNE_PAIR = 8,
    TUNE_FE_LEAN_INST = 9,
};
int tuning(TuningKey key);

hipError_t raise_dyn_lds(std::initializer_list<const void *> fns, int bytes);
hipError_t launch_update_ssh_f32(const MeshDev &m, const float *h, float *ssh, int nlev, int lpc, hipStream_t s);
hipError_t launch_permute_rows_f32(void *dst, const void *src, const int32_t *n2o, int64_t n, int K, int to_device,
                                   hipStream_t s);
hipError_t launch_halo_map_f32(float *buf, float *h, float *ssh, float *u, const uint32_t *map, int64_t n, int unpack,
                               hipStream_t s);
hipError_t launch_fe(const MeshDev &m, const FeArgs &a, int lpc, hipStream_t s);
hipError_t launch_curl2(const MeshDev &m, const double *u, double *vort, bool accum, hipStream_t s);
hipError_t launch_curl_f32(const MeshDev &m, const float *u, float *vort, bool accum, hipStream_t s);
hipError_t launch_operator(const MeshDev &m, const OpArgs &a, int lpc, hipStream_t s);
hipError_t launch_update_ssh(const MeshDev &m, const double *h, double *ssh, int nlev, int lpc, hipStream_t s);
hipError_t launch_permute_rows(double *dst, const double *src, const int32_t *n2o, int64_t n, int K, int to_device,
                               hipStream_t s);
hipError_t launch_sum_sq_serial(const double *a, int64_t n, double *out, hipStream_t s);
hipError_t launch_copy(double *dst, const double *src, int64_t n, hipStream_t s);
hipError_t launch_bw_copy(void *dst, const void *src, int64_t bytes, int nCUs, hipStream_t s);
hipError_t launch_bw_streams(void *buf, int64_t bytes, hipStream_t s);
hipError_t launch_bw_gather_n(const void *src, int64_t nRows, uint32_t rowB, int64_t nFetch, uint32_t *sink, int nCUs, hipStream_t s);
hipError_t launch_bw_read(const void *src, int64_t bytes, uint32_t *sink, int nCUs, hipStream_t s);
hipError_t launch_bw_gather(const void *src, int64_t bytes, uint32_t rowB, uint32_t *sink, int nCUs, hipStream_t s);
hipError_t launch_halo_map(double *buf, double *h, double *ssh, double *u, const uint32_t *map, int64_t n, int unpack,
                           hipStream_t s);
hipError_t launch_pack_rows(double *buf, const double *field, const int32_t *rows, int64_t n, int K, int unpack, hipStream_t s);

struct NlArgs {
    double *qv;
    double *fq;
    double *ke;
    double *zv;
    double *divc;
    double visc;
    const double *div4;
    const double *curl4;
    const double *coef4;
};
bool nl_stage_is_nl5(const MeshDev &m, int lpc, bool rowsOk, int form);
bool nl_patch_forms(const MeshDev &m, int lpc, int form);
hipError_t launch_nl_prepare(const MeshDev &m, const double *u, const double *h, const NlArgs &nl, int lpc, int form, hipStream_t s);
hipError_t launch_stage_nl(const MeshDev &m, const StageArgs &a, const NlArgs &nl, int lpc, bool rowsOk, int form, hipStream_t s);
struct D4Rows {
    const int32_t *start;
    const int32_t *row;
    const uint16_t *locC;
    const uint16_t *locV;
    int32_t maxRows;
};
int del4_path(const MeshDev &m, const D4Rows &r, int lpc, int form);
hipError_t launch_del4(const MeshDev &m, const D4Rows &r, const double *divc, const double *zv, double *div4, double *curl4, int path,
                       hipStream_t s);

struct TracerArgs {
    int nT, stage;
    int64_t stride;
    const double *pu, *ph;
    const double *hcur;
    const double *hnext;
    const double *pphi;
    const double *cphi;
    double *pphi_out;
    double *qn;
    double a, b;
    const double *kappa, *dvdc;
    const double *const *src;
    const double *kappa4, *lap;
};
struct TracerKernel {
    int form;
    size_t lds;
    int chunk;
};
TracerKernel tracer_kernel(const MeshDev &m, int lpc, int nT, bool generic, bool diff, bool bih);
hipError_t launch_tracers(const MeshDev &m, const TracerArgs &a, int lpc, bool generic, hipStream_t s);

struct TracerLapArgs {
    int nT;
    int64_t stride;
    const double *ph;
    const double *x;
    const double *kappa4, *dvdc;
    double *out;
// ... 124 lines not shown
```

mpas-ocean.jl_amd/csrc/kernels_common.hpp:

```cpp
#pragma once
#include <atomic>
#include <algorithm>
#include <hip/hip_runtime.h>

#include "kernels.hpp"

namespace moka {

constexpr int BLOCK = 256;

template <int LPC>
__device__ __forceinline__ double group_sum(double v)
{
#pragma unroll
    for (int s = LPC / 2; s >= 1; s >>= 1) v = v + __shfl_xor(v, s, 64);
    return v;
}

template <class T> using CP = const T __attribute__((address_space(4))) *;
template <class T> __device__ __forceinline__ CP<T> cptr(const T *p) { return (CP<T>)(uintptr_t)p; }

template <int LPC>
__device__ __forceinline__ int uniform_if_wave(int x)
{
// ... 117 lines not shown
                 "s_waitcnt lgkmcnt(0)"
                 : [o0] "=&v"(v[0]), [o1] "=&v"(v[1]), [o2] "=&v"(v[2]), [o3] "=&v"(v[3]), [o4] "=&v"(v[4]), [o5] "=&v"(v[5]), [o6] "=&v"(v[6]), [o7] "=&v"(v[7]), [o8] "=&v"(v[8]), [o9] "=&v"(v[9])
                 : [a0] "v"(ad[0]), [a1] "v"(ad[1]), [a2] "v"(ad[2]), [a3] "v"(ad[3]), [a4] "v"(ad[4]), [a5] "v"(ad[5]), [a6] "v"(ad[6]), [a7] "v"(ad[7]), [a8] "v"(ad[8]), [a9] "v"(ad[9])
                 : "memory");
}
template <>
__device__ __forceinline__ void lds_burst<14>(v4u_t (&v)[14], const uint32_t (&ad)[14])
{
    asm volatile("ds_read_b128 %[o0], %[a0]\n\t"
                 "ds_read_b128 %[o1], %[a1]\n\t"
                 "ds_read_b128 %[o2], %[a2]\n\t"
                 "ds_read_b128 %[o3], %[a3]\n\t"
                 "ds_read_b128 %[o4], %[a4]\n\t"
                 "ds_read_b128 %[o5], %[a5]\n\t"
                 "ds_read_b128 %[o6], %[a6]\n\t"
                 "ds_read_b128 %[o7], %[a7]\n\t"
                 "ds_read_b128 %[o8], %[a8]\n\t"
                 "ds_read_b128 %[o9], %[a9]\n\t"
                 "ds_read_b128 %[o10], %[a10]\n\t"
                 "ds_read_b128 %[o11], %[a11]\n\t"
                 "ds_read_b128 %[o12], %[a12]\n\t"
                 "ds_read_b128 %[o13], %[a13]\n\t"
                 "s_waitcnt lgkmcnt(0)"
                 : [o0] "=&v"(v[0]), [o1] "=&v"(v[1]), [o2] "=&v"(v[2]), [o3] "=&v"(v[3]), [o4] "=&v"(v[4]), [o5] "=&v"(v[5]), [o6] "=&v"(v[6]), [o7] "=&v"(v[7]), [o8] "=&v"(v[8]), [o9] "=&v"(v[9]), [o10] "=&v"(v[10]), [o11] "=&v"(v[11]), [o12] "=&v"(v[12]), [o13] "=&v"(v[13])
                 : [a0] "v"(ad[0]), [a1] "v"(ad[1]), [a2] "v"(ad[2]), [a3] "v"(ad[3]), [a4] "v"(ad[4]), [a5] "v"(ad[5]), [a6] "v"(ad[6]), [a7] "v"(ad[7]), [a8] "v"(ad[8]), [a9] "v"(ad[9]), [a10] "v"(ad[10]), [a11] "v"(ad[11]), [a12] "v"(ad[12]), [a13] "v"(ad[13])
                 : "memory");
}
__device__ __forceinline__ double2 glb_row2(glb_bytes_t p)
{
    const v2d_t v = *(const __attribute__((address_space(1))) v2d_t *)p;
    return make_double2(v.x, v.y);
}
__device__ __forceinline__ float4 glb_row4f(glb_bytes_t p)
{
    const v4f_t v = *(const __attribute__((address_space(1))) v4f_t *)p;
    return make_float4(v.x, v.y, v.z, v.w);
}

__device__ __forceinline__ void gstore2o(double *base, uint32_t off, double2 x)
{
#if defined(MOKA_EXP_WT_STORES)
    __builtin_amdgcn_raw_buffer_store_b128(__builtin_bit_cast(u32x4, x), make_rsrc(base, 0xFFFFFFFFu), (int)off, 0, 16);
#elif defined(MOKA_EXP_NT_STORES)
    __builtin_amdgcn_raw_buffer_store_b128(__builtin_bit_cast(u32x4, x), make_rsrc(base, 0xFFFFFFFFu), (int)off, 0, 2);
#elif defined(MOKA_EXP_NO_STORES)
    if (x.x == 1.2345e300) gstore2(base, off, x);
#else
    gstore2(base, off, x);
#endif
}

struct RecLds {
    uint32_t *eRec, *cRec;
    double *woe, *feoe, *g, *sdv, *invA, *rsum;
};

__device__ __forceinline__ RecLds rec_carve(unsigned char *smem, const ColMesh &m, int ME, int ME2, int maxOwnE, int maxOwnC)
{
    RecLds L;
    L.woe = reinterpret_cast<double *>(smem);
    L.feoe = L.woe + (size_t)maxOwnE * ME2;
    L.g = L.feoe + (size_t)maxOwnE * ME2;
    L.sdv = L.g + maxOwnE;
    L.invA = L.sdv + (size_t)maxOwnC * ME;
    L.rsum = L.invA + maxOwnC;
    L.eRec = reinterpret_cast<uint32_t *>(L.rsum + maxOwnC);
    L.cRec = L.eRec + (size_t)maxOwnE * m.EI;
    return L;
}

static inline int patch_grid(const MeshDev &m) { return 8 * ((m.nPatches + 7) / 8); }

inline int colp_mode(const StageArgs &a)
{
    if (a.feMode) {
        const bool lvl = a.pu_out && a.ph_out && a.ssh_out, noLvl = !a.pu_out && !a.ph_out && !a.ssh_out;
        const bool dia = a.tendU && a.tendH && a.F && a.div && a.hEdgeNew && a.areaCell, noDia = !a.tendU && !a.tendH && !a.F && !a.div && !a.hEdgeNew;
        const bool ok = (lvl || noLvl) && (dia || noDia) && (lvl || dia) && !a.cu && !a.ch && !a.nu_in && !a.nh_in && !a.nu_out && !a.nh_out &&
                        (a.feMode == 4 ? a.hEdgeOld != nullptr : a.feMode == 6 ? a.hPrev != nullptr : a.feMode == 5);
        return ok ? a.feMode : -1;
    }
    if (a.rkMode) {
        const bool p = a.pu_out && a.ph_out && a.ssh_out, c = a.cu && a.ch, n = a.nu_out && a.nh_out && a.ssh_out;
        if (a.rkMode == 7) return p && !c ? 7 : -1;
        if (a.rkMode == 8) return p && c ? 8 : -1;
        if (a.rkMode == 9) return n && c && a.nu_in && a.nh_in && a.q3u && a.q3h ? 9 : -1;
        return -1;
    }
    const bool outs = a.pu_out || a.ph_out || a.nu_out || a.nh_out;
    if (a.tendU && a.tendH && !outs && !a.ssh_out) return 0;
    if (a.tendU || a.tendH) return -1;
    if (!a.cu && !a.ch && !a.nu_in && !a.nh_in && a.pu_out && a.ph_out && a.nu_out && a.nh_out && a.ssh_out) return 1;
    if (a.cu && a.ch && a.nu_in && a.nh_in && a.pu_out && a.ph_out && a.nu_out && a.nh_out && a.ssh_out) return 2;
    if (a.nu_in && a.nh_in && !a.pu_out && !a.ph_out && a.nu_out && a.nh_out && a.ssh_out) return 3;
    return -1;
}

inline bool colp_lean(const StageArgs &a, int mode)
{
    return (mode == 5 || mode == 6) && a.pu_out && a.ph_out && a.ssh_out && !a.tendU && !a.tendH && !a.F && !a.div && !a.hEdgeNew;
}

inline size_t rec_lds_bytes(const MeshDev &md)
{
    return (size_t)md.maxOwnE * (2 * md.ME2 + 1) * 8 + (size_t)md.maxOwnC * (md.ME + 2) * 8 +
           ((size_t)md.maxOwnE * md.EI + (size_t)md.maxOwnC * md.CI) * 4 + 16;
}


__device__ __forceinline__ double rk13_combine(double c, double p2, double p3, double p4, double b4, double t)
{
    const double d2 = p2 - c, d3 = p3 - c, d4 = p4 - c;
    const double acc = (d2 + (d3 + d3)) + d4;
    return (c + acc * (1.0 / 3.0)) + b4 * t;
}

#define DISPATCH_LPC(lpc, CALL)                 \
    switch (lpc) {                              \
        case 1: return CALL(1);                 \
        case 2: return CALL(2);                 \
        case 4: return CALL(4);                 \
        case 8: return CALL(8);                 \
        case 16: return CALL(16);               \
        case 32: return CALL(32);               \
        default: return CALL(64);               \
    }

}
```

mpas-ocean.jl_amd/csrc/placement.hip:

```cpp
#include <algorithm>
#include <cmath>
#include <cstring>

#include "state.hpp"

using namespace mk;

namespace {

struct FieldSlot {
    int id;
    int set;
    int which;
    unsigned stages;
};
const FieldSlot kSlots[12] = {{6, 2, 0, 0xF}, {9, 3, 0, 0x6}, {3, 1, 0, 0xF}, {0, 0, 0, 0xF},
                              {7, 2, 1, 0xF}, {10, 3, 1, 0x6}, {4, 1, 1, 0xF}, {1, 0, 1, 0xF},
                              {8, 2, 2, 0xF}, {11, 3, 2, 0x6}, {5, 1, 2, 0x8}, {2, 0, 2, 0x1}};
constexpr int NSLOTS = 12;

LevelBufs &set_of(moka_state *st, int set) { return set == 0 ? st->lev[1] : set == 1 ? st->lev[0] : st->rk[set - 2]; }

void repoint(moka_state *st, double *oldp, double *newp)
{
    auto fix = [&](LevelBufs &b) {
        if (b.u == oldp) b.u = newp;
        if (b.h == oldp) b.h = newp;
        if (b.ssh == oldp) b.ssh = newp;
    };
    for (auto &b : st->lev) fix(b);
    for (auto &b : st->rk) fix(b);
    fix(st->spare);
    for (auto &b : st->phys) fix(b);
    for (void *&q : st->mem.ptrs) if (q == (void *)oldp) q = (void *)newp;
}

struct Timer {
    hipEvent_t ev[5] = {nullptr, nullptr, nullptr, nullptr, nullptr};
    ~Timer() { for (hipEvent_t e : ev) if (e) (void)hipEventDestroy(e); }
};

int time_stages(moka_state *st, Timer &T, int reps, double ms[4])
{
    moka_ctx *c = st->ctx;
    std::vector<float> v[4];
    for (int r = -1; r < reps; ++r) {
        for (int s = 1; s <= 4; ++s) {
            if (r >= 0) HIPCHK(c, hipEventRecord(T.ev[s - 1], c->stream));
            HIPCHK(c, run_stage(st, rk4_stage_args(st, s, 0.0, st->lev[1].ssh)));
            ++st->placementLaunches;
        }
        if (r < 0) continue;
        HIPCHK(c, hipEventRecord(T.ev[4], c->stream));
        HIPCHK(c, hipEventSynchronize(T.ev[4]));
        for (int s = 0; s < 4; ++s) {
            float t = 0.f;
            HIPCHK(c, hipEventElapsedTime(&t, T.ev[s], T.ev[s + 1]));
            v[s].push_back(t);
        }
    }
    for (int s = 0; s < 4; ++s) {
        std::sort(v[s].begin(), v[s].end());
        ms[s] = v[s][v[s].size() / 2];
    }
    return MOKA_OK;
}

double over(const double ms[4], unsigned stages)
{
    double t = 0.0;
    for (int s = 0; s < 4; ++s) if (stages >> s & 1u) t += ms[s];
    return t;
}

}

extern "C" {

int moka_state_optimize_placement(moka_state *st, int max_tries, double *ms_before, double *ms_after)
{
    if (!st) return fail(nullptr, MOKA_ERR_ARG, "state is NULL");
    moka_ctx *c = st->ctx;
    if (ms_before) *ms_before = 0.0;
    if (ms_after) *ms_after = 0.0;
    if (st->attached > 0)
        return fail(c, MOKA_ERR_UNSUPPORTED, "moka_state_optimize_placement: a halo or a tape of this state exists (they hold or have exported "
                                            "the arrays' addresses); call it before moka_halo_create / moka_tape_create");
    HIPCHK(c, hipSetDevice(c->device));
    st->placementLog.clear();
    st->placementLaunches = 0;
    int rc = ensure_rk_bufs(st);
    if (rc) return rc;
    if ((rc = flush_lazy(st, !(st->f32 && st->diagDirty), true))) return rc;
    const Plan &p = st->mesh->plan;
    const size_t sb = st->f32 ? 4 : 8;
    const size_t bytesU = (size_t)p.K * p.nE * sb, bytesH = (size_t)p.K * p.nC * sb, bytesS = (size_t)p.nC * sb;
    hipStream_t s = c->stream;
    Timer T;
    for (hipEvent_t &e : T.ev) HIPCHK(c, hipEventCreate(&e));

    void *save[3] = {nullptr, nullptr, nullptr};
    std::vector<std::pair<void *, size_t>> held;
    size_t heldBytes = 0;
    auto cleanup = [&]() {
        (void)hipStreamSynchronize(s);
        for (void *q : save) if (q) (void)hipFree(q);
        for (auto &h : held) (void)hipFree(h.first);
    };
    const size_t saveBytes[3] = {bytesU, bytesH, bytesS};
    for (int i = 0; i < 3; ++i)
        if (hipMalloc(&save[i], std::max<size_t>(saveBytes[i], 16)) != hipSuccess) {
            (void)hipGetLastError();
            cleanup();
            return fail(c, MOKA_ERR_ALLOC, "moka_state_optimize_placement: no memory to save the previous time level");
        }
    {
        const LevelBufs &B = st->lev[0];
        hipError_t e = hipMemcpyAsync(save[0], B.u, bytesU, hipMemcpyDeviceToDevice, s);
        if (e == hipSuccess) e = hipMemcpyAsync(save[1], B.h, bytesH, hipMemcpyDeviceToDevice, s);
        if (e == hipSuccess) e = hipMemcpyAsync(save[2], B.ssh, bytesS, hipMemcpyDeviceToDevice, s);
        if (e != hipSuccess) { cleanup(); return fail(c, MOKA_ERR_HIP, std::string("hipMemcpyAsync: ") + hipGetErrorString(e)); }
    }
    auto restore = [&]() -> hipError_t {
        const LevelBufs &B = st->lev[0];
        hipError_t e = hipMemcpyAsync(B.u, save[0], bytesU, hipMemcpyDeviceToDevice, s);
        if (e == hipSuccess) e = hipMemcpyAsync(B.h, save[1], bytesH, hipMemcpyDeviceToDevice, s);
        if (e == hipSuccess) e = hipMemcpyAsync(B.ssh, save[2], bytesS, hipMemcpyDeviceToDevice, s);
        if (e == hipSuccess) e = hipStreamSynchronize(s);
        return e;
    };
    constexpr int REPS = 5;
    double best[4];
// ... 95 lines not shown
```

mpas-ocean.jl_amd/csrc/state.hpp:

```cpp
#pragma once
#include <hip/hip_runtime.h>

#include <algorithm>
#include <initializer_list>
#include <map>
#include <string>
#include <utility>
#include <vector>

#include "kernels.hpp"
#include "moka_internal.hpp"

struct moka_ctx {
    int device = 0;
    hipStream_t stream = nullptr;
    hipStream_t comm = nullptr;
    hipEvent_t ev0 = nullptr, ev1 = nullptr;
    hipEvent_t evBoundary = nullptr, evInterior = nullptr, evHalo = nullptr;
    int variant = 0;
    int nCUs = 256;
    std::string err;
    bool stageTiming = false;
    std::vector<hipEvent_t> evPool;
    size_t evUsed = 0;
// ... 84 lines not shown
};

}

struct moka_mesh {
    moka_ctx *ctx = nullptr;
    moka::Plan plan;
    moka::MeshDev dev{};
    mk::DeviceAllocs mem;
    int lpc = 1;
    bool colOk = false;
    double *opBuf[4] = {nullptr, nullptr, nullptr, nullptr};
    size_t opBufElems = 0;
    const int32_t *opTVert = nullptr;
    const double *opTCoef = nullptr;
    const double *opESign = nullptr;
    int opTW = 0;
    std::map<std::pair<int, int>, std::pair<int, int>> rangeMax;
    const double *dvdc = nullptr;
    const int32_t *nLev = nullptr;
    moka::D4Rows d4{};
};

struct LevelBufs {
    double *ssh = nullptr, *u = nullptr, *h = nullptr;
};

struct moka_state {
    moka_ctx *ctx = nullptr;
    moka_mesh *mesh = nullptr;
    LevelBufs lev[2];
    double *hEdge[2] = {nullptr, nullptr};
    double *F = nullptr, *div = nullptr, *vort = nullptr, *tendU = nullptr, *tendH = nullptr;
    LevelBufs rk[2];
    LevelBufs spare;
    static constexpr int NPHYS = 5;
    LevelBufs phys[NPHYS];
    bool hEdgePrev = false;
    bool feLazy = false, feLazyStale = false;
    bool feForceEager = false;
    bool feLeanInteriorOnly = false;
    int feLazyBegin = 0, feLazyCount = -1;
    double *scalar = nullptr;
    bool sshConsistent = false;
    bool diagDirty = false;
    bool tendDirty = false;
    const double *lazyPu = nullptr, *lazyPh = nullptr;
    const void *lazyOwner = nullptr;
    bool f32 = false;
    bool nonlinear = false;
    int nlPhase = 0;
    double *nlQv = nullptr, *nlQe = nullptr, *nlKe = nullptr;
    int feFast = -1;
    double *nlZv = nullptr, *nlDiv = nullptr;
    double viscDel2 = 0.0;
    double *nlDiv4 = nullptr, *nlCurl4 = nullptr, *coef4 = nullptr;
    double viscDel4 = 0.0;
    int del4Path = 0;
    int halos = 0;
    int nTracers = 0;
    double *trPhi[2] = {nullptr, nullptr}, *trProv[2] = {nullptr, nullptr};
    int tracerPath = 0;
    std::vector<double> trKappa;
    double *trKappaDev = nullptr;
    std::vector<double> trKappa4;
    double *trKappa4Dev = nullptr, *trLap = nullptr;
    std::vector<double> trKappaV;
    double *trKappaVDev = nullptr, *trVmixScratch = nullptr;
    int vmixPath = 0;
    std::vector<double *> trVf;
    std::vector<char> trVfOn;
    std::vector<uint64_t> trVfGen;
    uint64_t trVfClock = 0;
    double **trVfDev = nullptr;
    std::vector<double *> trSrc;
    double **trSrcDev = nullptr;
    double momNuV = 0.0, momDrag = 0.0;
    double *momTau = nullptr, *momScratch = nullptr;
    bool momTauOn = false;
    double *momVf = nullptr;
    bool momVfOn = false;
    uint64_t momVfGen = 0;
    int momVmixPath = 0;
    mk::DeviceAllocs mem;
    int attached = 0;
    int dycoreTapes = 0;
    int forcedTapes = 0;
    int64_t forcedSteps = 0;
    std::vector<moka_placement_trial> placementLog;
    int64_t placementLaunches = 0;
};

namespace mk {

using namespace moka;

void state_attach(moka_state *st, bool halo = false);
bool state_detach(moka_state *st, bool halo = false);

inline bool default_stage_kernels(const moka_state *st)
{
    const int v = st->ctx->variant;
    return (v == 0 || v == 11) && st->mesh->lpc == 64 && st->mesh->colOk;
}
inline MeshDev launch_bounds(const moka_mesh *mm)
{
    MeshDev dev = mm->dev;
    dev.maxOwnE = std::max(mm->plan.maxOwnELaunch, 1); dev.maxOwnC = std::max(mm->plan.maxOwnCLaunch, 1);
    return dev;
}
inline bool mom_vmix_on(const moka_state *st)
{
    return (st->momVf ? st->momVfOn : st->momNuV != 0.0) || st->momDrag != 0.0 || (st->momTau && st->momTauOn);
}
inline const double *mom_vmix_field(const moka_state *st) { return st->momVf && st->momVfOn ? st->momVf : nullptr; }
inline double mom_vmix_nu(const moka_state *st) { return st->momVf ? 0.0 : st->momNuV; }
inline int nl_form(const moka_ctx *ctx) { return ctx->variant == 4 ? 1 : ctx->variant == 3 ? 3 : 0; }

int ensure_op_bufs(moka_mesh *m);
const int32_t *perm_of(const moka_mesh *m, int kind);
int put_rows(moka_mesh *m, double *dst, const double *host, int kind, int64_t n, int K, bool f32 = false);
int get_rows(moka_mesh *m, double *host, const double *src, int kind, int64_t n, int K, bool f32 = false);
int ensure_rk_bufs(moka_state *st);
int ensure_spare(moka_state *st);
LevelBufs &fe_new_level(moka_state *st);
void fe_rotate_levels(moka_state *st);
int flush_lazy(moka_state *st, bool diag, bool tend);
hipError_t run_stage(moka_state *st, const StageArgs &g, int pBegin = 0, int pCount = -1, hipStream_t on = nullptr, int tail = -1);
StageArgs rk4_stage_args(moka_state *st, int s, double dt, const double *ssh0);
LevelBufs &rk4_stage_output(moka_state *st, int s);
int rk4_begin(moka_state *st, const double **ssh0);
void rk4_end(moka_state *st);
bool rk13_usable(const moka_state *st);
StageArgs rk13_stage_args(moka_state *st, int s, double dt, const double *ssh0);
void rk13_end(moka_state *st);
FeArgs fe_args(moka_state *st, int ops, int flags, double dt);
StageArgs fe_stage_args(moka_state *st, const FeArgs &a, int flags);
bool fe_stage_path(const moka_state *st, int flags);
bool fe_lean(const moka_state *st, int flags);
int fe_begin(moka_state *st, int flags);
void fe_end(moka_state *st, int flags, bool stageKernel, bool lean, bool prevMode);
int step_rk4(moka_state *st, double dt, moka_tracer_tape *rec);
int momentum_vmix(moka_state *st, double *u, const double *h, double dt);
hipError_t tracer_stage(moka_state *st, int s, const StageArgs &g);
int tracer_vmix(moka_mesh *mm, moka_ctx *ctx, int nT, const double *h, double *x, const double *kv, const double *const *fld, double dt,
                double *scratch, bool reverse, int *path, const int32_t *gslot = nullptr, const double *p_new = nullptr, double *D = nullptr);
bool vfield_on(const moka_state *st, int j);
double vmix_coefficient(const moka_state *st, const std::vector<double> &kv, int j);

}
```

mpas-ocean.jl_amd/moka_hip/lib.py:

```python
from __future__ import annotations

import ctypes as C
import os
import subprocess

import numpy as np

PKG_DIR = os.path.dirname(os.path.dirname(os.path.abspath(__file__)))
LIB_PATH = os.environ.get("MOKA_HIP_LIB") or os.path.join(PKG_DIR, "libmoka_hip.so")

_i32p = C.POINTER(C.c_int32)
_f64p = C.POINTER(C.c_double)

OK = 0
ERR_ARG, ERR_HIP, ERR_NO_DEVICE, ERR_ALLOC, ERR_UNSUPPORTED, ERR_COMM = -1, -2, -3, -4, -5, -6
ORDER_DEFAULT, ORDER_NONE, ORDER_RCM, ORDER_RCB = 0, 1, 2, 3
TRACER_GRAD_KAPPA, TRACER_GRAD_KAPPA4 = 1, 2
VGRAD_INTERFACE, VGRAD_CELL, VGRAD_PROFILE = 0, 1, 2
FORCED_GRAD_STRESS, FORCED_GRAD_VISCOSITY, FORCED_GRAD_DRAG = 1, 2, 4
CELL, EDGE, VERTEX = 0, 1, 2
(F_SSH, F_NORMAL_VELOCITY, F_LAYER_THICKNESS, F_LAYER_THICKNESS_EDGE, F_THICKNESS_FLUX,
 F_VELOCITY_DIV_CELL, F_RELATIVE_VORTICITY, F_TEND_NORMAL_VELOCITY, F_TEND_LAYER_THICKNESS) = range(9)
FE_STALE_HEDGE, FE_ACCUM_VORT, FE_LEVEL1_ONLY, FE_REFERENCE_COMPAT = 1, 2, 4, 7
FORWARD_EULER, RUNGE_KUTTA_4 = 0, 1


class MokaError(RuntimeError):

    def __init__(self, code, msg):
        super().__init__(f"libmoka_hip error {code}: {msg}")
        self.code = code


class MeshDesc(C.Structure):
    _fields_ = [
        ("nCells", C.c_int32), ("nEdges", C.c_int32), ("nVertices", C.c_int32),
        ("maxEdges", C.c_int32), ("maxEdges2", C.c_int32), ("vertexDegree", C.c_int32),
        ("nVertLevels", C.c_int32), ("edgeSignOnVertexLD", C.c_int32),
        ("xCell", _f64p), ("yCell", _f64p), ("zCell", _f64p),
        ("nEdgesOnCell", _i32p), ("edgesOnCell", _i32p), ("edgeSignOnCell", _i32p), ("areaCell", _f64p),
        ("cellsOnEdge", _i32p), ("verticesOnEdge", _i32p), ("nEdgesOnEdge", _i32p), ("edgesOnEdge", _i32p),
        ("weightsOnEdge", _f64p), ("dvEdge", _f64p), ("dcEdge", _f64p), ("fEdge", _f64p),
        ("edgesOnVertex", _i32p), ("cellsOnVertex", _i32p), ("edgeSignOnVertex", _i32p), ("areaTriangle", _f64p),
        ("maxLevelEdgeTop", _i32p), ("restingThicknessSum", _f64p),
        ("ordering", C.c_int32), ("patch_cells", C.c_int32),
        ("cellClass", _i32p),
        ("stateBytes", C.c_int32),
        ("kiteAreasOnVertex", _f64p), ("fVertex", _f64p),
    ]


class HaloStats(C.Structure):
    _fields_ = [("steps", C.c_int64), ("exchanges", C.c_int64), ("boundary_launches", C.c_int64), ("interior_launches", C.c_int64),
                ("host_step_ms", C.c_double), ("host_signal_wait_ms", C.c_double), ("host_flag_store_ms", C.c_double),
                ("host_wait_ms", C.c_double), ("boundary_launch_ms", C.c_double), ("interior_launch_ms", C.c_double)]


class PlacementTrial(C.Structure):
    _fields_ = [("field", C.c_int32), ("ms_old", C.c_double), ("ms_new", C.c_double), ("kept", C.c_int32)]


class MeshInfo(C.Structure):
    _fields_ = [
        ("nCells", C.c_int32), ("nEdges", C.c_int32), ("nVertices", C.c_int32), ("nVertLevels", C.c_int32),
        ("ordering", C.c_int32), ("patch_cells", C.c_int32), ("nPatches", C.c_int32),
        ("maxEdgesUsed", C.c_int32), ("maxEdges2Used", C.c_int32), ("lanesPerColumn", C.c_int32),
        ("meshBytesDevice", C.c_int64), ("cellBandwidth", C.c_int64),
        ("maxPatchRows", C.c_int32), ("ldsBytesPerBlock", C.c_int32),
        ("maxPatchCells", C.c_int32), ("maxPatchEdges", C.c_int32),
    ]

    def as_dict(self):
        return {n: getattr(self, n) for n, _ in self._fields_}


EXPORTS = [
    "moka_version", "moka_ctx_create", "moka_ctx_destroy", "moka_last_error", "moka_sync",
    "moka_timer_start", "moka_timer_stop",
    "moka_plan_create", "moka_plan_destroy", "moka_plan_info", "moka_plan_permutation", "moka_plan_patch_ranges", "moka_plan_array",
    "moka_mesh_create", "moka_mesh_destroy", "moka_mesh_info_get",
    "moka_gradient_on_edge", "moka_divergence_on_cell", "moka_curl_on_vertex", "moka_interpolate_cell2edge",
    "moka_state_create", "moka_state_destroy", "moka_state_upload", "moka_state_download",
    "moka_advance_time_levels", "moka_diagnostic_compute", "moka_compute_normal_velocity_tendency",
    "moka_compute_layer_thickness_tendency", "moka_tendencies", "moka_step_fe", "moka_step_rk4", "moka_run",
    "moka_sum_sq", "moka_set_kernel_variant", "moka_kernel_variant_available", "moka_stage_timing", "moka_stage_timing_read",
    "moka_ctx_streams", "moka_halo_create", "moka_halo_destroy", "moka_halo_buffer_elems", "moka_halo_pack",
    "moka_halo_unpack", "moka_rk4_dist_begin", "moka_rk4_dist_stage", "moka_rk4_dist_end",
    "moka_plan_class_ranges", "moka_mesh_class_ranges", "moka_mesh_permutation", "moka_halo_direct_available", "moka_halo_set_overlap", "moka_halo_pack_fields", "moka_halo_unpack_fields",
    "moka_tape_record_rk4", "moka_tape_commit_rk4", "moka_adjoint_rk4_stage_fields", "moka_adjoint_rk4_stage",
    "moka_tape_record_fe", "moka_tape_commit_fe", "moka_adjoint_fe_step_fields", "moka_adjoint_fe_step",
    "moka_halo_export", "moka_halo_connect", "moka_halo_push_begin", "moka_halo_push_signal", "moka_halo_push_wait",
    "moka_rk4_dist_stage_launch", "moka_rk4_dist_step", "moka_fe_dist_launch", "moka_fe_dist_end", "moka_fe_dist_step",
    "moka_set_nonlinear", "moka_last_fe_path", "moka_set_viscosity_del2", "moka_set_viscosity_del4", "moka_state_del4_path", "moka_tape_create", "moka_tape_destroy", "moka_step_fe_taped", "moka_step_rk4_taped", "moka_adjoint_seed_sum_sq_ssh", "moka_adjoint_sweep",
    "moka_adjoint_download",
    "moka_mark", "moka_marks_reset", "moka_marks_read", "moka_bw_probe", "moka_bw_probe_streams", "moka_bw_probe_reread", "moka_bw_probe_gather_big", "moka_ctx_pci_bus_id", "moka_halo_set_acquire", "moka_set_tuning", "moka_get_tuning", "moka_rk4_dist_parts_available", "moka_adjoint_rk4_stage_part", "moka_adjoint_rk4_parts_available", "moka_adjoint_rk4_stage_out_fields",
    "moka_gradient_on_edge_vjp", "moka_gradient_on_edge_jvp", "moka_divergence_on_cell_vjp", "moka_divergence_on_cell_jvp",
    "moka_curl_on_vertex_vjp", "moka_curl_on_vertex_jvp", "moka_fe_lazy_pending",
    "moka_state_optimize_placement", "moka_state_placement_log", "moka_state_download_rows",
    "moka_halo_stats_enable", "moka_halo_stats_read", "moka_halo_set_stream_flags", "moka_state_array_address", "moka_state_placement_launches",
    "moka_state_rk4_streams",
    "moka_set_tracers", "moka_tracer_upload", "moka_tracer_download", "moka_state_tracer_path",
    "moka_set_tracer_diffusion", "moka_tracer_diffusion",
    "moka_set_tracer_biharmonic", "moka_tracer_biharmonic",
    "moka_set_tracer_vertical_diffusion", "moka_tracer_vertical_diffusion", "moka_state_tracer_vmix_path", "moka_tracer_adjoint_vmix_path",
    "moka_tracer_source_upload", "moka_tracer_source_download", "moka_tracer_has_source",
    "moka_tracer_vertical_field_upload", "moka_tracer_vertical_field_download", "moka_tracer_has_vertical_field",
    "moka_set_vertical_viscosity", "moka_vertical_viscosity", "moka_surface_stress_upload", "moka_surface_stress_download",
    "moka_has_surface_stress", "moka_state_momentum_vmix_path",
    "moka_vertical_viscosity_field_upload", "moka_vertical_viscosity_field_download", "moka_has_vertical_viscosity_field",
    "moka_tracer_adjoint_want_source_gradient", "moka_tracer_adjoint_source_download",
    "moka_tracer_adjoint_want_diffusivity_gradient", "moka_tracer_adjoint_diffusivity_gradient",
    "moka_tracer_adjoint_diffusivity_density_download",
    "moka_tracer_adjoint_want_vertical_gradient", "moka_tracer_adjoint_vertical_gradient",
    "moka_tracer_adjoint_vertical_density_download",
    "moka_tracer_tape_create", "moka_tracer_tape_destroy", "moka_step_rk4_tracer_taped", "moka_tracer_tape_steps",
    "moka_tracer_adjoint_seed", "moka_tracer_adjoint_sweep", "moka_tracer_adjoint_download", "moka_tracer_adjoint_path",
    "moka_forced_tape_create", "moka_forced_tape_destroy", "moka_step_rk4_forced_taped", "moka_forced_adjoint_seed_sum_sq_ssh",
    "moka_forced_adjoint_seed", "moka_forced_adjoint_sweep", "moka_forced_adjoint_download", "moka_forced_adjoint_want_gradient",
    "moka_forced_adjoint_density_download", "moka_forced_adjoint_gradient", "moka_forced_tape_vmix_path",
    "moka_forced_adjoint_want_viscosity_field_gradient", "moka_forced_adjoint_viscosity_field_density_download",
]


def build(force: bool = False) -> str:
    if force:
        subprocess.check_call(["make", "-C", PKG_DIR, "--no-print-directory", "clean"])
    subprocess.check_call(["make", "-C", PKG_DIR, "--no-print-directory", "-j4"])
    return LIB_PATH


_lib = None


def lib():
    global _lib
    if _lib is not None:
        return _lib
    if not os.path.exists(LIB_PATH):
        raise MokaError(ERR_NO_DEVICE, f"{LIB_PATH} is missing: build it with `make -C {PKG_DIR}` "
                                       "(there is no CPU fallback for the HIP path)")
    try:
        import torch
    except ImportError:
        pass
    L = C.CDLL(LIB_PATH)
    vp = C.c_void_p
    L.moka_version.restype = C.c_char_p
    L.moka_last_error.restype = C.c_char_p
    L.moka_last_error.argtypes = [vp]
    L.moka_ctx_create.argtypes = [C.c_int, C.POINTER(vp)]
    L.moka_ctx_destroy.argtypes = [vp]
    L.moka_ctx_destroy.restype = None
    L.moka_sync.argtypes = [vp]
    L.moka_timer_start.argtypes = [vp]
    L.moka_timer_stop.argtypes = [vp, C.POINTER(C.c_float)]
    L.moka_plan_create.argtypes = [C.POINTER(MeshDesc), C.POINTER(vp)]
    L.moka_plan_destroy.argtypes = [vp]
    L.moka_plan_destroy.restype = None
    L.moka_plan_info.argtypes = [vp, C.POINTER(MeshInfo)]
    L.moka_plan_permutation.argtypes = [vp, C.c_int, _i32p]
    L.moka_plan_patch_ranges.argtypes = [vp, _i32p, _i32p, _i32p]
    L.moka_plan_array.argtypes = [vp, C.c_int, C.POINTER(vp), C.POINTER(C.c_int64)]
    L.moka_mesh_create.argtypes = [vp, C.POINTER(MeshDesc), C.POINTER(vp)]
    L.moka_mesh_destroy.argtypes = [vp]
    L.moka_mesh_destroy.restype = None
    L.moka_mesh_info_get.argtypes = [vp, C.POINTER(MeshInfo)]
    L.moka_gradient_on_edge.argtypes = [vp, _f64p, _f64p]
    L.moka_divergence_on_cell.argtypes = [vp, _f64p, _f64p, _f64p]
    L.moka_curl_on_vertex.argtypes = [vp, _f64p, _f64p]
    L.moka_interpolate_cell2edge.argtypes = [vp, _f64p, _f64p, C.c_int]
    L.moka_gradient_on_edge_vjp.argtypes = [vp, _f64p, _f64p]
    L.moka_gradient_on_edge_jvp.argtypes = [vp, _f64p, _f64p]
    L.moka_divergence_on_cell_vjp.argtypes = [vp, _f64p, _f64p, _f64p]
    L.moka_divergence_on_cell_jvp.argtypes = [vp, _f64p, _f64p, _f64p]
    L.moka_curl_on_vertex_vjp.argtypes = [vp, _f64p, _f64p]
    L.moka_curl_on_vertex_jvp.argtypes = [vp, _f64p, _f64p]
    L.moka_state_create.argtypes = [vp, vp, C.POINTER(vp)]
    L.moka_state_destroy.argtypes = [vp]
    L.moka_state_destroy.restype = None
    L.moka_state_optimize_placement.argtypes = [vp, C.c_int, _f64p, _f64p]
    L.moka_state_placement_launches.argtypes = [vp]
    L.moka_state_rk4_streams.argtypes = [vp]
    L.moka_state_placement_launches.restype = C.c_int64
    L.moka_state_placement_log.argtypes = [vp, C.c_int32, C.POINTER(PlacementTrial), _i32p]
    L.moka_state_array_address.argtypes = [vp, C.c_int, C.c_int, C.POINTER(C.c_uint64)]
    L.moka_state_download_rows.argtypes = [vp, C.c_int, C.c_int, C.c_int64, _i32p, _f64p]
    L.moka_state_upload.argtypes = [vp, C.c_int, C.c_int, _f64p]
    L.moka_state_download.argtypes = [vp, C.c_int, C.c_int, _f64p]
    L.moka_advance_time_levels.argtypes = [vp, C.c_int]
    L.moka_diagnostic_compute.argtypes = [vp, C.c_int]
    L.moka_compute_normal_velocity_tendency.argtypes = [vp, C.c_int]
    L.moka_compute_layer_thickness_tendency.argtypes = [vp, C.c_int]
    L.moka_tendencies.argtypes = [vp]
    L.moka_step_fe.argtypes = [vp, C.c_double, C.c_int]
    L.moka_step_rk4.argtypes = [vp, C.c_double]
    L.moka_run.argtypes = [vp, C.c_int, C.c_double, C.c_int64, C.c_int]
    L.moka_sum_sq.argtypes = [vp, C.c_int, C.c_int, _f64p]
    L.moka_set_kernel_variant.argtypes = [vp, C.c_int]
    L.moka_kernel_variant_available.argtypes = [C.c_int]
    L.moka_stage_timing.argtypes = [vp, C.c_int]
    L.moka_stage_timing_read.argtypes = [vp, C.POINTER(C.c_double), C.POINTER(C.c_int64)]
    L.moka_ctx_streams.argtypes = [vp, C.POINTER(vp), C.POINTER(vp)]
    i64p = C.POINTER(C.c_int64)
    L.moka_halo_create.argtypes = [vp, C.c_int32, _i32p, i64p, _i32p, i64p, _i32p, i64p, _i32p, i64p,
                                   C.c_int32, C.c_int32, C.POINTER(vp)]
    L.moka_halo_destroy.argtypes = [vp]
    L.moka_halo_set_stream_flags.argtypes = [vp, C.c_int]
    L.moka_halo_stats_enable.argtypes = [vp, C.c_int]
    L.moka_halo_stats_read.argtypes = [vp, C.POINTER(HaloStats)]
    L.moka_halo_destroy.restype = None
    L.moka_halo_buffer_elems.argtypes = [vp, C.POINTER(C.c_int64), C.POINTER(C.c_int64)]
    L.moka_halo_pack.argtypes = [vp, C.c_int, vp]
    L.moka_halo_unpack.argtypes = [vp, C.c_int, vp]
    L.moka_rk4_dist_begin.argtypes = [vp, C.c_double]
    L.moka_rk4_dist_stage.argtypes = [vp, C.c_int, C.c_int]
    L.moka_rk4_dist_parts_available.argtypes = [vp]
    L.moka_rk4_dist_end.argtypes = [vp]
    L.moka_plan_class_ranges.argtypes = [vp, C.c_int32, C.POINTER(C.c_int32), _i32p, _i32p, _i32p]
    L.moka_mesh_class_ranges.argtypes = [vp, C.c_int32, C.POINTER(C.c_int32), _i32p, _i32p, _i32p]
    L.moka_mesh_permutation.argtypes = [vp, C.c_int, _i32p]
    L.moka_halo_direct_available.argtypes = [vp]
    L.moka_halo_set_overlap.argtypes = [vp, C.c_int]
    L.moka_halo_set_acquire.argtypes = [vp, C.c_int]
    L.moka_halo_pack_fields.argtypes = [vp, vp, vp, vp, vp]
    L.moka_halo_unpack_fields.argtypes = [vp, vp, vp, vp, vp]
    L.moka_tape_record_rk4.argtypes = [vp, C.c_int, C.c_int]
    L.moka_tape_commit_rk4.argtypes = [vp, C.c_double]
    L.moka_adjoint_rk4_stage_fields.argtypes = [vp, C.c_int, C.POINTER(vp), C.POINTER(vp), C.POINTER(vp)]
    L.moka_adjoint_rk4_stage.argtypes = [vp, C.c_int]
    L.moka_adjoint_rk4_stage_part.argtypes = [vp, C.c_int, C.c_int]
    L.moka_adjoint_rk4_parts_available.argtypes = [vp]
    L.moka_adjoint_rk4_stage_out_fields.argtypes = [vp, C.c_int, C.POINTER(vp), C.POINTER(vp), C.POINTER(vp)]
    L.moka_tape_record_fe.argtypes = [vp, C.c_int, C.c_int]
    L.moka_tape_commit_fe.argtypes = [vp, C.c_double, C.c_int]
    L.moka_adjoint_fe_step_fields.argtypes = [vp, C.POINTER(vp), C.POINTER(vp), C.POINTER(vp)]
    L.moka_adjoint_fe_step.argtypes = [vp]
    L.moka_halo_export.argtypes = [vp, C.c_int32, C.c_int32, C.POINTER(HaloPeerInfo)]
    L.moka_halo_connect.argtypes = [vp, C.c_int32, C.POINTER(HaloPeerInfo), C.c_int32]
    L.moka_halo_push_begin.argtypes = [vp, C.c_int]
    L.moka_halo_push_signal.argtypes = [vp]
    L.moka_halo_push_wait.argtypes = [vp, C.c_double]
    L.moka_rk4_dist_stage_launch.argtypes = [vp, C.c_int]
    L.moka_rk4_dist_step.argtypes = [vp, C.c_double, TRANSPORT_FN, vp, vp, vp, C.c_double]
    L.moka_fe_dist_launch.argtypes = [vp, C.c_double, C.c_int, C.c_int]
    L.moka_fe_dist_end.argtypes = [vp]
    L.moka_fe_dist_step.argtypes = [vp, C.c_double, C.c_int, TRANSPORT_FN, vp, vp, vp, C.c_double]
    L.moka_set_nonlinear.argtypes = [vp, C.c_int]
    L.moka_last_fe_path.argtypes = [vp]
    L.moka_fe_lazy_pending.argtypes = [vp]
    L.moka_set_viscosity_del2.argtypes = [vp, C.c_double]
    L.moka_set_viscosity_del4.argtypes = [vp, C.c_double, vp]
    L.moka_state_del4_path.argtypes = [vp]
    L.moka_set_tracers.argtypes = [vp, C.c_int32]
    L.moka_tracer_upload.argtypes = [vp, C.c_int32, C.c_int, vp]
    L.moka_tracer_download.argtypes = [vp, C.c_int32, C.c_int, vp]
    L.moka_state_tracer_path.argtypes = [vp]
    L.moka_set_tracer_diffusion.argtypes = [vp, vp]
    L.moka_tracer_diffusion.argtypes = [vp, C.c_int32, C.POINTER(C.c_double)]
    L.moka_set_tracer_biharmonic.argtypes = [vp, vp]
    L.moka_tracer_biharmonic.argtypes = [vp, C.c_int32, C.POINTER(C.c_double)]
    L.moka_set_tracer_vertical_diffusion.argtypes = [vp, vp]
    L.moka_tracer_vertical_diffusion.argtypes = [vp, C.c_int32, C.POINTER(C.c_double)]
    L.moka_state_tracer_vmix_path.argtypes = [vp]
    L.moka_tracer_adjoint_vmix_path.argtypes = [vp]
    L.moka_tracer_tape_create.argtypes = [vp, C.c_int64, C.POINTER(vp)]
# ... 202 lines not shown
```

Measured before the change: 9.122 billion.

## Store RK4 stage-1 accumulator as byte residuals against a prediction

Adds new stage kernel modes 12 and 13 and enables them by default through a new tuning key. In RK4 stage 1 the next-level accumulator is stored as an 8-bit integer difference in its bit pattern from a prediction c + (p1 - c)/3, which stage 2 can rebuild from data it already reads. Rows where any value's residual does not fit fall back to full f64 storage, marked by a per-row flag. The aim is to cut the f64 write and read of the intermediate accumulator between stages, in exchange for extra residual and flag buffers, extra per-element integer work, a per-row flag load, and branching.

```diff
diff --git a/include/moka_hip.h b/include/moka_hip.h
--- a/include/moka_hip.h
+++ b/include/moka_hip.h
@@ -218,6 +218,7 @@
 int moka_set_kernel_variant(moka_ctx *ctx, int variant);
 int moka_set_tuning(int key, int value);
 int moka_get_tuning(int key, int *value);
+int moka_state_coded_rows(moka_state *st, int64_t *coded, int64_t *raw);
 int moka_state_rk4_streams(const moka_state *st);
 int moka_stage_timing(moka_ctx *ctx, int enable);
 int moka_stage_timing_read(moka_ctx *ctx, double ms[4], int64_t *steps);
diff --git a/mpas-ocean.jl_amd/csrc/api.hip b/mpas-ocean.jl_amd/csrc/api.hip
--- a/mpas-ocean.jl_amd/csrc/api.hip
+++ b/mpas-ocean.jl_amd/csrc/api.hip
@@ -24,6 +24,7 @@
     std::atomic<int> value;
     TuningEntry(int def, int m, int x) : mask(m), max(x), value(def) {}
     bool accepts(int v) const { return mask ? (v & ~mask) == 0 : v >= 0 && v <= max; }
+    bool known() const { return mask != 0 || max >= 0; }
 };
 static TuningEntry g_tuning[] = {
     {0, 0, -1},
@@ -35,6 +36,9 @@
     {0, 0, INT_MAX},
     {0, 0, 1},
     {1 << 0 | 1 << 1 | 1 << 7, 0xf | 7 << 7 | 1 << 16, 0},
+    {1, 0, 1},
+    {0, 0, -1},
+    {0, 0, -1},
     {1, 0, 1},
 };
 constexpr int N_TUNING = sizeof(g_tuning) / sizeof(g_tuning[0]);
@@ -370,7 +374,7 @@
 
 int moka_set_tuning(int key, int value)
 {
-    if (key < 1 || key >= N_TUNING) return fail(nullptr, MOKA_ERR_ARG, "unknown tuning key");
+    if (key < 1 || key >= N_TUNING || !g_tuning[key].known()) return fail(nullptr, MOKA_ERR_ARG, "unknown tuning key");
     if (!g_tuning[key].accepts(value)) return fail(nullptr, MOKA_ERR_ARG, "tuning key " + std::to_string(key) + ": value names no kernel instance");
     g_tuning[key].value.store(value);
     return MOKA_OK;
@@ -379,7 +383,7 @@
 int moka_get_tuning(int key, int *value)
 {
     if (!value) return fail(nullptr, MOKA_ERR_ARG, "value is NULL");
-    if (key < 1 || key >= N_TUNING) return fail(nullptr, MOKA_ERR_ARG, "unknown tuning key");
+    if (key < 1 || key >= N_TUNING || !g_tuning[key].known()) return fail(nullptr, MOKA_ERR_ARG, "unknown tuning key");
     *value = g_tuning[key].value.load();
     return MOKA_OK;
 }
diff --git a/mpas-ocean.jl_amd/csrc/api_state.hip b/mpas-ocean.jl_amd/csrc/api_state.hip
--- a/mpas-ocean.jl_amd/csrc/api_state.hip
+++ b/mpas-ocean.jl_amd/csrc/api_state.hip
@@ -332,7 +332,7 @@
     return MOKA_OK;
 }
 
-StageArgs rk4_stage_args(moka_state *st, int s, double dt, const double *ssh0)
+StageArgs rk4_stage_args(moka_state *st, int s, double dt, const double *ssh0, bool coded)
 {
     const double a[3] = {dt / 2., dt / 2., dt};
     const double b[4] = {dt / 6., dt / 3., dt / 3., dt / 6.};
@@ -352,6 +352,11 @@
         g.pu = R1.u; g.ph = R1.h; g.ssh = R1.ssh; g.cu = A.u; g.ch = A.h; g.nu_in = B.u; g.nh_in = B.h;
         g.ssh_out = B.ssh; g.a = 0.0;
     }
+    if (coded && s <= 2) {
+        g.rkMode = s == 1 ? 12 : 13;
+        g.resU = st->codeResU; g.resH = st->codeResH; g.flagU = st->codeFlagU; g.flagH = st->codeFlagH;
+        g.third = 1.0 / 3.0;
+    }
     return g;
 }
 
@@ -394,6 +399,30 @@
     if (st->nonlinear)
         return nl_stage_is_nl5(mm->dev, mm->lpc, mm->plan.ldsOk, nl_form(st->ctx));
     return default_stage_kernels(st) && rec2c_supported(launch_bounds(mm));
+}
+
+bool coded_usable(const moka_state *st)
+{
+    if (!tuning(TUNE_CODED) || st->f32 || st->nonlinear || st->nTracers > 0) return false;
+    const moka_mesh *mm = st->mesh;
+    if (mm->plan.nPatchesLaunch != mm->plan.nPatches) return false;
+    return default_stage_kernels(st) && rec2c_supported(launch_bounds(mm));
+}
+
+bool coded_begin(moka_state *st, bool capturing)
+{
+    if (!coded_usable(st) || rk13_usable(st)) return false;
+    if (st->codeResU) return true;
+    if (capturing) return false;
+    const Plan &p = st->mesh->plan;
+    const size_t m = st->mem.mark();
+    if (st->mem.alloc(&st->codeResU, (size_t)p.K * p.nE) || st->mem.alloc(&st->codeResH, (size_t)p.K * p.nC) ||
+        st->mem.alloc(&st->codeFlagU, (size_t)p.nE) || st->mem.alloc(&st->codeFlagH, (size_t)p.nC)) {
+        st->mem.rollback(m);
+        st->codeResU = st->codeResH = st->codeFlagU = st->codeFlagH = nullptr;
+        return false;
+    }
+    return true;
 }
 
 StageArgs rk13_stage_args(moka_state *st, int s, double dt, const double *ssh0)
@@ -468,9 +497,11 @@
         return hipEventRecord(c->evPool[c->evUsed++], c->stream);
     };
     const bool s13 = rk13_usable(st);
+    const bool coded = coded_begin(st, cap != hipStreamCaptureStatusNone);
+    st->codedLast = coded;
     for (int s = 1; s <= 4; ++s) {
         if (timed) HIPCHK(c, stamp());
-        const StageArgs g = s13 ? rk13_stage_args(st, s, dt, ssh0) : rk4_stage_args(st, s, dt, ssh0);
+        const StageArgs g = s13 ? rk13_stage_args(st, s, dt, ssh0) : rk4_stage_args(st, s, dt, ssh0, coded);
         HIPCHK(c, run_stage(st, g));
         if (st->nTracers > 0) HIPCHK(c, tracer_stage(st, s, g));
         if (s == 4 && vmix && st->mesh->plan.K >= 2 && dt != 0.0)
diff --git a/mpas-ocean.jl_amd/csrc/inspect.hip b/mpas-ocean.jl_amd/csrc/inspect.hip
--- a/mpas-ocean.jl_amd/csrc/inspect.hip
+++ b/mpas-ocean.jl_amd/csrc/inspect.hip
@@ -100,3 +100,19 @@
     *address = (uint64_t)(uintptr_t)q;
     return MOKA_OK;
 }
+
+extern "C" int moka_state_coded_rows(moka_state *st, int64_t *coded, int64_t *raw)
+{
+    if (!st || !coded || !raw) return fail(st ? st->ctx : nullptr, MOKA_ERR_ARG, "NULL argument");
+    *coded = *raw = 0;
+    if (!st->codedLast || !st->codeFlagU) return MOKA_OK;
+    moka_ctx *c = st->ctx;
+    HIPCHK(c, hipSetDevice(c->device));
+    const Plan &p = st->mesh->plan;
+    std::vector<unsigned char> f((size_t)p.nE + (size_t)p.nC);
+    HIPCHK(c, hipMemcpyAsync(f.data(), st->codeFlagU, (size_t)p.nE, hipMemcpyDeviceToHost, c->stream));
+    HIPCHK(c, hipMemcpyAsync(f.data() + p.nE, st->codeFlagH, (size_t)p.nC, hipMemcpyDeviceToHost, c->stream));
+    HIPCHK(c, hipStreamSynchronize(c->stream));
+    for (unsigned char x : f) ++*(x ? raw : coded);
+    return MOKA_OK;
+}
diff --git a/mpas-ocean.jl_amd/csrc/kernels.hip b/mpas-ocean.jl_amd/csrc/kernels.hip
--- a/mpas-ocean.jl_amd/csrc/kernels.hip
+++ b/mpas-ocean.jl_amd/csrc/kernels.hip
@@ -31,8 +31,10 @@
     const uint32_t e0B = (uint32_t)e0 * rowB, nOwnB = (uint32_t)nOwnE * rowB;
     double *Lvw = reinterpret_cast<double *>(smem + recBytes + (size_t)maxOwnE * rowB);
     uint32_t *Lvo = reinterpret_cast<uint32_t *>(Lvw + (size_t)m.maxOwnV * 3);
-    constexpr bool LEAN = MODE >= 10;
+    constexpr bool LEAN = MODE == 10 || MODE == 11;
     constexpr int BASE = LEAN ? MODE - 5 : MODE;
+    constexpr bool ENC = MODE == 12, DEC = MODE == 13;
+    constexpr int RK = ENC ? 1 : DEC ? 2 : MODE;
     constexpr bool FE = BASE >= 4 && BASE <= 6, STALE = BASE == 4, PREV = BASE == 6;
     int v0 = 0, nOwnV = 0;
     if constexpr (FE) {
@@ -124,15 +126,18 @@
     uint32_t pOff = 0;
     int pC = 0;
     bool pend = false;
+    uint32_t pR = 0, fl = 0, flN = 0;
+    bool pRaw = true;
     auto flush_cell = [&]() {
         if (act) {
-            if constexpr (MODE == 0) gstore2o(a.tendH, pOff, pA);
-            if constexpr (MODE == 1 || MODE == 2) {
+            if constexpr (RK == 0) gstore2o(a.tendH, pOff, pA);
+            if constexpr (RK == 1 || RK == 2) {
                 gstore2o(a.ph_out, pOff, pA);
-                gstore2o(a.nh_out, pOff, pB);
-            }
-            if constexpr (MODE == 3 || MODE == 9) gstore2o(a.nh_out, pOff, pB);
-            if constexpr (MODE == 7 || MODE == 8) gstore2o(a.ph_out, pOff, pA);
+                if (!ENC || pRaw) gstore2o(a.nh_out, pOff, pB);
+                if constexpr (ENC) if (!pRaw) gstore_res2(a.resH, pOff, pR);
+            }
+            if constexpr (RK == 3 || RK == 9) gstore2o(a.nh_out, pOff, pB);
+            if constexpr (RK == 7 || RK == 8) gstore2o(a.ph_out, pOff, pA);
             if constexpr (LEAN) gstore2o(a.ph_out, pOff, pA);
             if constexpr (FE && !LEAN) {
                 if (a.ph_out) gstore2o(a.ph_out, pOff, pA);
@@ -140,9 +145,11 @@
                 if (a.div) gstore2o(a.div, pOff, pD);
             }
         }
-        if constexpr (MODE != 0)
+        if constexpr (RK != 0)
             if (l == 0 && (!FE || LEAN || a.ssh_out)) a.ssh_out[pC] = pS;
+        if constexpr (ENC) if (l == 0) a.flagH[pC] = pRaw ? 1 : 0;
     };
+    if constexpr (DEC) if (grp < nOwnC) fl = a.flagH[c0 + grp];
 #pragma nounroll
     for (int ci = grp; ci < nOwnC; ci += NG) {
         const int c = c0 + ci;
@@ -172,14 +179,20 @@
                 uv[i] = __builtin_bit_cast(double2, raw[i]);
                 if (!cached[i]) uv[i] = glb_row2(puG + goff[i]);
             }
-            if constexpr (MODE == 2 || MODE == 8 || MODE == 9) cur = gload2(a.ch, own);
-            if constexpr (MODE == 2 || MODE == 3 || MODE == 9) nin = gload2(a.nh_in, own);
-            if constexpr (MODE == 9) q3 = gload2(a.q3h, own);
+            if constexpr (RK == 2 || RK == 8 || RK == 9) cur = gload2(a.ch, own);
+            if constexpr (DEC) {
+                pR = gload_res2(a.resH, own);
+                if (fl) nin = gload2(a.nh_in, own);
+                flN = ci + NG < nOwnC ? a.flagH[c + NG] : 0u;
+            } else if constexpr (RK == 2 || RK == 3 || RK == 9) nin = gload2(a.nh_in, own);
+            if constexpr (RK == 9) q3 = gload2(a.q3h, own);
         }
         double area = 1.0;
         if constexpr (FE && !LEAN) if (a.div) area = a.areaCell[c];
         __builtin_amdgcn_s_waitcnt(0x0F70);
         if (pend) flush_cell();
+        if constexpr (DEC)
+            if (act && !fl) nin = make_double2(coded_decode(pR & 0xffu, cur.x, hc.x, a.third), coded_decode(pR >> 8, cur.y, hc.y, a.third));
         double2 t = make_double2(0.0, 0.0);
         const bool plain = __builtin_amdgcn_ballot_w64(!(mask == (1u << ME) - 1u && all)) == 0;
         double2 dv = make_double2(0.0, 0.0);
@@ -217,25 +230,32 @@
             }
         }
         double2 hs = make_double2(0.0, 0.0);
+        bool fits = true;
         if (act) {
-            if constexpr (MODE == 0) pA = t;
-            if constexpr (MODE == 1 || MODE == 2) {
-                const double2 hcur = MODE == 2 ? cur : hc;
-                const double2 nb = MODE == 2 ? nin : hcur;
+            if constexpr (RK == 0) pA = t;
+            if constexpr (RK == 1 || RK == 2) {
+                const double2 hcur = RK == 2 ? cur : hc;
+                const double2 nb = RK == 2 ? nin : hcur;
                 hs = make_double2(hcur.x + a.a * t.x, hcur.y + a.a * t.y);
                 pA = hs;
                 pB = make_double2(nb.x + a.b * t.x, nb.y + a.b * t.y);
-            }
-            if constexpr (MODE == 3) {
+                if constexpr (ENC) {
+                    bool fx, fy;
+                    const uint64_t dx = coded_residual(pB.x, hc.x, pA.x, a.third, fx), dy = coded_residual(pB.y, hc.y, pA.y, a.third, fy);
+                    pR = ((uint32_t)dx & 0xffu) | (((uint32_t)dy & 0xffu) << 8);
+                    fits = fx && fy;
+                }
+            }
+            if constexpr (RK == 3) {
                 hs = make_double2(nin.x + a.b * t.x, nin.y + a.b * t.y);
                 pB = hs;
             }
-            if constexpr (MODE == 7 || MODE == 8) {
-                const double2 hcur = MODE == 8 ? cur : hc;
+            if constexpr (RK == 7 || RK == 8) {
+                const double2 hcur = RK == 8 ? cur : hc;
                 hs = make_double2(hcur.x + a.a * t.x, hcur.y + a.a * t.y);
                 pA = hs;
             }
-            if constexpr (MODE == 9) {
+            if constexpr (RK == 9) {
                 hs = make_double2(rk13_combine(cur.x, nin.x, q3.x, hc.x, a.b, t.x), rk13_combine(cur.y, nin.y, q3.y, hc.y, a.b, t.y));
                 pB = hs;
             }
@@ -248,7 +268,7 @@
                 }
             }
         }
-        if constexpr (MODE != 0) {
+        if constexpr (RK != 0) {
 #pragma unroll
             for (int sft = 16; sft >= 1; sft >>= 1) {
                 const double ox = __shfl_xor(hs.x, sft, 32), oy = __shfl_xor(hs.y, sft, 32);
@@ -256,6 +276,8 @@
             }
             pS = (hs.x + hs.y) - L.rsum[ci];
         }
+        if constexpr (ENC) pRaw = half_wave_any(!fits);
+        if constexpr (DEC) fl = flN;
         pOff = own;
         pC = c;
         pend = true;
@@ -264,13 +286,14 @@
     pend = false;
     auto flush_edge = [&]() {
         if (act) {
-            if constexpr (MODE == 0) gstore2o(a.tendU, pOff, pA);
-            if constexpr (MODE == 1 || MODE == 2) {
+            if constexpr (RK == 0) gstore2o(a.tendU, pOff, pA);
+            if constexpr (RK == 1 || RK == 2) {
                 gstore2o(a.pu_out, pOff, pA);
-                gstore2o(a.nu_out, pOff, pB);
-            }
-            if constexpr (MODE == 3 || MODE == 9) gstore2o(a.nu_out, pOff, pB);
-            if constexpr (MODE == 7 || MODE == 8) gstore2o(a.pu_out, pOff, pA);
+                if (!ENC || pRaw) gstore2o(a.nu_out, pOff, pB);
+                if constexpr (ENC) if (!pRaw) gstore_res2(a.resU, pOff, pR);
+            }
+            if constexpr (RK == 3 || RK == 9) gstore2o(a.nu_out, pOff, pB);
+            if constexpr (RK == 7 || RK == 8) gstore2o(a.pu_out, pOff, pA);
             if constexpr (LEAN) gstore2o(a.pu_out, pOff, pA);
             if constexpr (FE && !LEAN) {
                 if (a.pu_out) gstore2o(a.pu_out, pOff, pA);
@@ -279,7 +302,9 @@
                 if (a.hEdgeNew) gstore2o(a.hEdgeNew, pOff, pE);
             }
         }
+        if constexpr (ENC) if (l == 0) a.flagU[pC] = pRaw ? 1 : 0;
     };
+    if constexpr (DEC) fl = grp < nOwnE ? a.flagU[e0 + grp] : 0u;
 
 #pragma nounroll
     for (int ei = grp; ei < nOwnE; ei += NG) {
@@ -310,11 +335,15 @@
                 uv[i] = __builtin_bit_cast(double2, raw[i]);
                 if (!cached[i]) uv[i] = glb_row2(puG + goff[i]);
             }
-            if constexpr (MODE == 2 || MODE == 8 || MODE == 9) cur = gload2(a.cu, own);
-            if constexpr (MODE == 2 || MODE == 3 || MODE == 9) nin = gload2(a.nu_in, own);
-            if constexpr (MODE == 9) q3 = gload2(a.q3u, own);
+            if constexpr (RK == 2 || RK == 8 || RK == 9) cur = gload2(a.cu, own);
+            if constexpr (DEC) {
+                pR = gload_res2(a.resU, own);
+                if (fl) nin = gload2(a.nu_in, own);
+                flN = ei + NG < nOwnE ? a.flagU[e + NG] : 0u;
+            } else if constexpr (RK == 2 || RK == 3 || RK == 9) nin = gload2(a.nu_in, own);
+            if constexpr (RK == 9) q3 = gload2(a.q3u, own);
             if constexpr (FE && !LEAN) {
-                if (a.hEdgeNew || (MODE == 5 && a.F)) {
+                if (a.hEdgeNew || (RK == 5 && a.F)) {
                     hx = gload2(a.ph, r[ME2] * rowB + voff);
                     hy = gload2(a.ph, r[ME2 + 1] * rowB + voff);
                 }
@@ -332,6 +361,7 @@
         if (pend) flush_edge();
         const double ds = __shfl(sv, 1, 32) - __shfl(sv, 0, 32);
         const bool plain = __builtin_amdgcn_ballot_w64(!(mask == (1u << ME2) - 1u && mlt >= K)) == 0;
+        bool fits = true;
         if (act) {
             const bool ax = k0 < mlt, ay = k0 + 1 < mlt;
             double2 t = make_double2(0.0, 0.0);
@@ -354,23 +384,34 @@
                     if (on && ay) t.y += py;
                 }
             }
-            if constexpr (MODE == 0) pA = t;
-            if constexpr (MODE == 1) {
+            if constexpr (RK == 0) pA = t;
+            if constexpr (RK == 1) {
                 const double2 up = ubuf2[(size_t)ei * K2 + l];
                 pA = make_double2(up.x + a.a * t.x, up.y + a.a * t.y);
                 pB = make_double2(up.x + a.b * t.x, up.y + a.b * t.y);
-            }
-            if constexpr (MODE == 2) {
+                if constexpr (ENC) {
+                    bool fx, fy;
+                    const uint64_t dx = coded_residual(pB.x, up.x, pA.x, a.third, fx), dy = coded_residual(pB.y, up.y, pA.y, a.third, fy);
+                    pR = ((uint32_t)dx & 0xffu) | (((uint32_t)dy & 0xffu) << 8);
+                    fits = fx && fy;
+                }
+            }
+            if constexpr (RK == 2) {
+                if constexpr (DEC)
+                    if (!fl) {
+                        const double2 p1 = ubuf2[(size_t)ei * K2 + l];
+                        nin = make_double2(coded_decode(pR & 0xffu, cur.x, p1.x, a.third), coded_decode(pR >> 8, cur.y, p1.y, a.third));
+                    }
                 pA = make_double2(cur.x + a.a * t.x, cur.y + a.a * t.y);
                 pB = make_double2(nin.x + a.b * t.x, nin.y + a.b * t.y);
             }
-            if constexpr (MODE == 3) pB = make_double2(nin.x + a.b * t.x, nin.y + a.b * t.y);
-            if constexpr (MODE == 7) {
+            if constexpr (RK == 3) pB = make_double2(nin.x + a.b * t.x, nin.y + a.b * t.y);
+            if constexpr (RK == 7) {
                 const double2 up = ubuf2[(size_t)ei * K2 + l];
                 pA = make_double2(up.x + a.a * t.x, up.y + a.a * t.y);
             }
-            if constexpr (MODE == 8) pA = make_double2(cur.x + a.a * t.x, cur.y + a.a * t.y);
-            if constexpr (MODE == 9) {
+            if constexpr (RK == 8) pA = make_double2(cur.x + a.a * t.x, cur.y + a.a * t.y);
+            if constexpr (RK == 9) {
                 const double2 up = ubuf2[(size_t)ei * K2 + l];
                 pB = make_double2(rk13_combine(cur.x, nin.x, q3.x, up.x, a.b, t.x), rk13_combine(cur.y, nin.y, q3.y, up.y, a.b, t.y));
             }
@@ -387,6 +428,9 @@
                 pB = t;
             }
         }
+        if constexpr (ENC) pRaw = half_wave_any(!fits);
+        if constexpr (DEC) fl = flN;
+        if constexpr (ENC) pC = e;
         pOff = own;
         pend = true;
     }
@@ -1359,6 +1403,8 @@
         case 9: hipLaunchKernelGGL((k_stage_rec2c<ME, ME2, 9, NT>), g, b, lds, s, m, a, mE, mC); return true;
         case 10: hipLaunchKernelGGL((k_stage_rec2c<ME, ME2, 10, NT>), g, b, lds, s, m, a, mE, mC); return true;
         case 11: hipLaunchKernelGGL((k_stage_rec2c<ME, ME2, 11, NT>), g, b, lds, s, m, a, mE, mC); return true;
+        case 12: hipLaunchKernelGGL((k_stage_rec2c<ME, ME2, 12, NT>), g, b, lds, s, m, a, mE, mC); return true;
+        case 13: hipLaunchKernelGGL((k_stage_rec2c<ME, ME2, 13, NT>), g, b, lds, s, m, a, mE, mC); return true;
     }
     return false;
 }
@@ -1397,7 +1443,7 @@
         hipLaunchKernelGGL((k_stage_rec2c<ME, ME2, M, 512>), g, b, lds, s, m, a, mE, mC);                               \
         return hipGetLastError();
     switch (mode) {
-        PAIR_CASE(0) PAIR_CASE(1) PAIR_CASE(2) PAIR_CASE(3) PAIR_CASE(7) PAIR_CASE(8) PAIR_CASE(9)
+        PAIR_CASE(0) PAIR_CASE(1) PAIR_CASE(2) PAIR_CASE(3) PAIR_CASE(7) PAIR_CASE(8) PAIR_CASE(9) PAIR_CASE(12) PAIR_CASE(13)
     }
 #undef PAIR_CASE
     return hipErrorNotSupported;
@@ -1447,7 +1493,8 @@
     const size_t lds = rec2c_lds_bytes(md) + (a.vort ? vert_lds_bytes(md) : 0);
     if (mode < 0 || md.K > 64 || (md.K & 1) || lds > 64 * 1024 || md.maxOwnC < 1 || md.maxOwnE < 1) return hipErrorNotSupported;
     const int pair = tuning(TUNE_PAIR);
-    if (((pair >> mode) & 1) && md.tailPatch < 0 && (md.nPatches >= 4096 || ((pair >> 16) & 1)) && md.nPatches >= 2 &&
+    const int pairBit = mode == 12 ? 1 : mode == 13 ? 2 : mode;
+    if (((pair >> pairBit) & 1) && md.tailPatch < 0 && (md.nPatches >= 4096 || ((pair >> 16) & 1)) && md.nPatches >= 2 &&
         md.ME == 6 && md.ME2 == 10) {
         MeshDev two = md;
         two.maxOwnE = 2 * md.maxOwnE; two.maxOwnC = 2 * md.maxOwnC;
diff --git a/mpas-ocean.jl_amd/csrc/kernels.hpp b/mpas-ocean.jl_amd/csrc/kernels.hpp
--- a/mpas-ocean.jl_amd/csrc/kernels.hpp
+++ b/mpas-ocean.jl_amd/csrc/kernels.hpp
@@ -26,6 +26,8 @@
     int accumVort;
     int rkMode;
     const double *q3u, *q3h;
+    unsigned char *resU, *resH, *flagU, *flagH;
+    double third;
 };
 
 struct ColMesh {
@@ -88,6 +90,7 @@
     TUNE_RK13 = 7,
     TUNE_PAIR = 8,
     TUNE_FE_LEAN_INST = 9,
+    TUNE_CODED = 12,
 };
 int tuning(TuningKey key);
 
diff --git a/mpas-ocean.jl_amd/csrc/kernels_common.hpp b/mpas-ocean.jl_amd/csrc/kernels_common.hpp
--- a/mpas-ocean.jl_amd/csrc/kernels_common.hpp
+++ b/mpas-ocean.jl_amd/csrc/kernels_common.hpp
@@ -223,6 +223,9 @@
     }
     if (a.rkMode) {
         const bool p = a.pu_out && a.ph_out && a.ssh_out, c = a.cu && a.ch, n = a.nu_out && a.nh_out && a.ssh_out;
+        const bool coded = p && n && a.resU && a.resH && a.flagU && a.flagH;
+        if (a.rkMode == 12) return coded && !c && !a.nu_in && !a.nh_in ? 12 : -1;
+        if (a.rkMode == 13) return coded && c && a.nu_in && a.nh_in ? 13 : -1;
         if (a.rkMode == 7) return p && !c ? 7 : -1;
         if (a.rkMode == 8) return p && c ? 8 : -1;
         if (a.rkMode == 9) return n && c && a.nu_in && a.nh_in && a.q3u && a.q3h ? 9 : -1;
@@ -256,6 +259,36 @@
     return (c + acc * (1.0 / 3.0)) + b4 * t;
 }
 
+__device__ __forceinline__ double pred(double c, double p1, double third) { return c + (p1 - c) * third; }
+__device__ __forceinline__ uint64_t coded_pred_bits(double c, double p1, double third)
+{
+    const double p = pred(c, p1, third);
+    return __builtin_bit_cast(uint64_t, p != p ? c : p);
+}
+__device__ __forceinline__ uint64_t coded_residual(double n, double c, double p1, double third, bool &fits)
+{
+    const uint64_t d = __builtin_bit_cast(uint64_t, n) - coded_pred_bits(c, p1, third);
+    fits = d + 127u <= 254u;
+    return d;
+}
+__device__ __forceinline__ double coded_decode(uint32_t byte, double c, double p1, double third)
+{
+    return __builtin_bit_cast(double, coded_pred_bits(c, p1, third) + (uint64_t)(int64_t)(int8_t)byte);
+}
+__device__ __forceinline__ void gstore_res2(unsigned char *base, uint32_t rowOff8, uint32_t two)
+{
+    *reinterpret_cast<uint16_t *>(base + (rowOff8 >> 3)) = (uint16_t)two;
+}
+__device__ __forceinline__ uint32_t gload_res2(const unsigned char *base, uint32_t rowOff8)
+{
+    return *reinterpret_cast<const uint16_t *>(base + (rowOff8 >> 3));
+}
+__device__ __forceinline__ bool half_wave_any(bool vote)
+{
+    const uint64_t b = __builtin_amdgcn_ballot_w64(vote);
+    return (uint32_t)(b >> (threadIdx.x & 32u)) != 0u;
+}
+
 #define DISPATCH_LPC(lpc, CALL)                 \
     switch (lpc) {                              \
         case 1: return CALL(1);                 \
diff --git a/mpas-ocean.jl_amd/csrc/placement.hip b/mpas-ocean.jl_amd/csrc/placement.hip
--- a/mpas-ocean.jl_amd/csrc/placement.hip
+++ b/mpas-ocean.jl_amd/csrc/placement.hip
@@ -44,10 +44,11 @@
 {
     moka_ctx *c = st->ctx;
     std::vector<float> v[4];
+    const bool coded = coded_begin(st, false);
     for (int r = -1; r < reps; ++r) {
         for (int s = 1; s <= 4; ++s) {
             if (r >= 0) HIPCHK(c, hipEventRecord(T.ev[s - 1], c->stream));
-            HIPCHK(c, run_stage(st, rk4_stage_args(st, s, 0.0, st->lev[1].ssh)));
+            HIPCHK(c, run_stage(st, rk4_stage_args(st, s, 0.0, st->lev[1].ssh, coded)));
             ++st->placementLaunches;
         }
         if (r < 0) continue;
diff --git a/mpas-ocean.jl_amd/csrc/state.hpp b/mpas-ocean.jl_amd/csrc/state.hpp
--- a/mpas-ocean.jl_amd/csrc/state.hpp
+++ b/mpas-ocean.jl_amd/csrc/state.hpp
@@ -190,6 +190,8 @@
     bool momVfOn = false;
     uint64_t momVfGen = 0;
     int momVmixPath = 0;
+    unsigned char *codeResU = nullptr, *codeResH = nullptr, *codeFlagU = nullptr, *codeFlagH = nullptr;
+    bool codedLast = false;
     mk::DeviceAllocs mem;
     int attached = 0;
     int dycoreTapes = 0;
@@ -235,7 +237,9 @@
 void fe_rotate_levels(moka_state *st);
 int flush_lazy(moka_state *st, bool diag, bool tend);
 hipError_t run_stage(moka_state *st, const StageArgs &g, int pBegin = 0, int pCount = -1, hipStream_t on = nullptr, int tail = -1);
-StageArgs rk4_stage_args(moka_state *st, int s, double dt, const double *ssh0);
+StageArgs rk4_stage_args(moka_state *st, int s, double dt, const double *ssh0, bool coded = false);
+bool coded_usable(const moka_state *st);
+bool coded_begin(moka_state *st, bool capturing);
 LevelBufs &rk4_stage_output(moka_state *st, int s);
 int rk4_begin(moka_state *st, const double **ssh0);
 void rk4_end(moka_state *st);
diff --git a/mpas-ocean.jl_amd/moka_hip/lib.py b/mpas-ocean.jl_amd/moka_hip/lib.py
--- a/mpas-ocean.jl_amd/moka_hip/lib.py
+++ b/mpas-ocean.jl_amd/moka_hip/lib.py
@@ -98,7 +98,7 @@
     "moka_curl_on_vertex_vjp", "moka_curl_on_vertex_jvp", "moka_fe_lazy_pending",
     "moka_state_optimize_placement", "moka_state_placement_log", "moka_state_download_rows",
     "moka_halo_stats_enable", "moka_halo_stats_read", "moka_halo_set_stream_flags", "moka_state_array_address", "moka_state_placement_launches",
-    "moka_state_rk4_streams",
+    "moka_state_rk4_streams", "moka_state_coded_rows",
     "moka_set_tracers", "moka_tracer_upload", "moka_tracer_download", "moka_state_tracer_path",
     "moka_set_tracer_diffusion", "moka_tracer_diffusion",
     "moka_set_tracer_biharmonic", "moka_tracer_biharmonic",
@@ -181,6 +181,7 @@
     L.moka_state_optimize_placement.argtypes = [vp, C.c_int, _f64p, _f64p]
     L.moka_state_placement_launches.argtypes = [vp]
     L.moka_state_rk4_streams.argtypes = [vp]
+    L.moka_state_coded_rows.argtypes = [vp, C.POINTER(C.c_int64), C.POINTER(C.c_int64)]
     L.moka_state_placement_launches.restype = C.c_int64
     L.moka_state_placement_log.argtypes = [vp, C.c_int32, C.POINTER(PlacementTrial), _i32p]
     L.moka_state_array_address.argtypes = [vp, C.c_int, C.c_int, C.POINTER(C.c_uint64)]
```

New measurement: 9.258 billion, median of 6. 1.01x the previous value.
